# OpenPPL/ppq

Measured on AMD Instinct MI355X. Metric: calibration samples/sec (RuntimeCalibrationPass, KL 2048-bin, ResNet-50 INT8), higher is better.
Workload: dtype f32; 1 GPU; ResNet-50 topology (53 Conv + 1 Gemm, BN folded, seeded He init), RuntimeCalibrationPass kl 2048 bins, per-tensor INT8 activations, per-channel INT8 weights, 279 batches x 32 x 3x224x224 per GPU; samples=8928, batch=32, observed_tensors=72, rccl_ranks=1, async_observe=False, cache_params=False, channels_last=False, fuse_params=True, batch_observations=True, reuse_activations=False, replayed_batches=0, hip_graph=auto, graph_replays=0, miopen_find=False

## Files before the change

### include/ppq_hip.h

```cpp
#ifndef PPQ_HIP_H_
#define PPQ_HIP_H_

#include <stdint.h>

#ifdef __cplusplus
extern "C" {
#endif

typedef enum {
    PPQHIP_OK = 0,
    PPQHIP_ERR_INVALID_VALUE = -1,
    PPQHIP_ERR_UNSUPPORTED = -2,
    PPQHIP_ERR_HIP = -3
} ppqhip_status;

#define PPQHIP_ABI_VERSION 4

const char* ppqhip_last_error(void);
int ppqhip_version(void);
int ppqhip_device_arch(char* buf, int n);

int ppqhip_fq_linear_t(const float* x, const float* scale, const float* offset, float* out,
                       int64_t n, int clip_min, int clip_max, int rounding, void* stream);

// ... 49 lines not shown
    int64_t n, num_channel, elem_per_channel;
    int32_t clip_min, clip_max;
} ppqhip_lsq_job;
int ppqhip_fq_linear_c_bwd_multi(const ppqhip_lsq_job* jobs, int num_jobs, int rounding, void* stream);

int ppqhip_fq_float_t(const float* x, const float* scale, const float* offset, float* out,
                      int64_t n, int exponent, int mantissa, float clip_min, float clip_max,
                      int rounding, void* stream);

int ppqhip_fq_float_c(const float* x, const float* scale, const float* offset, float* out,
                      int64_t n, int64_t num_channel, int64_t elem_per_channel,
                      int exponent, int mantissa, float clip_min, float clip_max,
                      int rounding, void* stream);

typedef struct ppqhip_float_search_job {
    const float* x;
    int64_t rows, row_len;
    int32_t exponent, mantissa;
    float clip_min, clip_max;
} ppqhip_float_search_job;
int64_t ppqhip_float_scale_search_table_bytes(int num_jobs);
int ppqhip_float_scale_search(const ppqhip_float_search_job* jobs, int num_jobs, const float* candidates,
                              int num_candidates, int rounding, void* device_table, double* out, void* stream);

typedef struct ppqhip_fq_float_job {
    const float* x;
    const float* scale;
    const float* offset;
    float* out;
    int64_t n, num_channel, elem_per_channel;
    int32_t exponent, mantissa;
    float clip_min, clip_max;
} ppqhip_fq_float_job;
int64_t ppqhip_fq_float_multi_table_bytes(int num_jobs);
int ppqhip_fq_float_multi(const ppqhip_fq_float_job* jobs, int num_jobs, int rounding, void* device_table,
                          int upload, void* stream);

int ppqhip_fq_float_c_bwd(const float* x, const float* scale, const float* offset,
                          const float* grad_y, float* grad_x, float* grad_s, int64_t n,
                          int64_t num_channel, int64_t elem_per_channel,
                          int exponent, int mantissa, float clip_min, float clip_max,
                          int rounding, void* stream);

int64_t ppqhip_hist_workspace_bytes(int64_t n, int64_t num_bins);
int ppqhip_hist_sym_t(const float* x, int64_t n, float hist_scale, int clip_outliers,
                      int32_t* hist, int64_t num_bins, void* workspace, void* stream);

int ppqhip_hist_asym_t(const float* x, int64_t n, float min_value, float max_value,
                       int clip_outliers, int32_t* hist, int64_t num_bins, void* workspace,
                       void* stream);

int ppqhip_hist_sym_c(const float* x, int64_t n, int64_t num_channel, int64_t elem_per_channel,
                      float hist_scale, int clip_outliers, int32_t* hist, int64_t num_bins,
                      void* stream);

int ppqhip_hist_sym_c_scales(const float* x, int64_t n, int64_t num_channel, int64_t elem_per_channel,
                             const float* hist_scales, int clip_outliers, int32_t* hist,
                             int64_t num_bins, void* stream);
int ppqhip_hist_asym_c_ranges(const float* x, int64_t n, int64_t num_channel, int64_t elem_per_channel,
                              const float* mins, const float* maxs, int clip_outliers, int32_t* hist,
                              int64_t num_bins, void* stream);

int64_t ppqhip_quantile_workspace_bytes(int64_t n);
int ppqhip_quantile_t(const float* x, int64_t n, float q, float* dest, uint32_t* hint, void* workspace,
                      void* stream);

typedef struct ppqhip_quantile_job {
    const float* x;
    float* dest;
    uint32_t* hint;
    int64_t n;
} ppqhip_quantile_job;
int64_t ppqhip_quantile_multi_workspace_bytes(int num_jobs, int64_t total_elems);
int ppqhip_quantile_t_multi(const ppqhip_quantile_job* jobs, int num_jobs, float q, void* workspace,
                            void* stream);
void ppqhip_quantile_debug_layout(int64_t* out);
void ppqhip_quantile_hot_layout(int64_t* out);

int ppqhip_isotone_t(const float* x, int64_t n, float* dest, void* workspace, void* stream);

int64_t ppqhip_minmax_workspace_bytes(int64_t n);
int ppqhip_minmax_t(const float* x, int64_t n, float* minmax, void* workspace, void* stream);

int ppqhip_minmax_c(const float* x, int64_t n, int64_t num_channel, int64_t elem_per_channel,
                    float* mins, float* maxs, void* stream);

typedef struct ppqhip_minmax_c_job {
    const float* x;
    float* mins;
    float* maxs;
    int64_t n, num_channel, elem_per_channel;
    int32_t fresh, reserved;
} ppqhip_minmax_c_job;
int ppqhip_minmax_c_multi(const ppqhip_minmax_c_job* jobs, int num_jobs, void* stream);

int ppqhip_channel_sum(const float* x, int64_t n, int64_t num_channel, int64_t elem_per_channel,
                       double* sums, void* stream);

int64_t ppqhip_hist_rows(void);
int ppqhip_hist_sym_t_rows(const float* x, int64_t n, float hist_scale, int clip_outliers,
                           int32_t* rows, int64_t num_bins, void* stream);
int ppqhip_hist_asym_t_rows(const float* x, int64_t n, float min_value, float max_value,
                            int clip_outliers, int32_t* rows, int64_t num_bins, void* stream);
typedef struct ppqhip_minmax_job {
    const float* x;
    float* slots;
    int64_t n;
} ppqhip_minmax_job;
int ppqhip_minmax_t_slots_multi(const ppqhip_minmax_job* jobs, int num_jobs, void* stream);

typedef struct ppqhip_hist_job {
    const float* x;
    int32_t* rows;
    int64_t n;
    float p0, p1;
} ppqhip_hist_job;
int ppqhip_hist_t_rows_multi(const ppqhip_hist_job* jobs, int num_jobs, int asymmetric,
                             int clip_outliers, int64_t num_bins, void* stream);
int ppqhip_hist_rows_finish(const int32_t* rows, int64_t num_bins, int32_t* hist, void* stream);
int ppqhip_check_bin_rule(const float* x, int64_t n, float min_value, float hist_scale, int asymmetric, uint64_t* out, void* stream);
int64_t ppqhip_minmax_slots(void);
int ppqhip_minmax_t_slots(const float* x, int64_t n, float* slots, void* stream);
int ppqhip_minmax_slots_finish(const float* slots, float* minmax, void* stream);

float ppqhip_mse_loss_host(const int64_t* hist, int64_t num_bins, int start, int step, int end);

int64_t ppqhip_mse_search_workspace_bytes(int64_t num_hist);
int ppqhip_mse_search(const int32_t* hist, int64_t num_hist, int64_t num_bins,
                      const double* hist_scale, const double* min_value,
                      int quant_min, int quant_max, int symmetrical, int32_t* best,
                      void* workspace, void* stream);

int64_t ppqhip_kl_num_candidates(int64_t num_bins, int num_of_bits);
int ppqhip_kl_losses(const int32_t* hist, int64_t num_hist, int64_t num_bins, int num_of_bits,
                     double* losses, void* stream);

int ppqhip_tensor_clip_t(const float* value, const float* reference, const float* limit,
                         float* out, int64_t n, void* stream);
int ppqhip_tensor_clip_c(const float* value, const float* reference, const float* limit,
                         float* out, int64_t n, int64_t num_channel, int64_t elem_per_channel,
                         void* stream);
int ppqhip_rounding_loss(const float* x, const float* scale, const float* offset, float* out,
                         int64_t n, int64_t num_channel, int64_t elem_per_channel,
                         int clip_min, int clip_max, int rounding, void* stream);
int ppqhip_rounding_loss_bwd(const float* x, const float* dy, const float* scale,
                             const float* offset, float* dx, int64_t n, int64_t num_channel,
                             int64_t elem_per_channel, int clip_min, int clip_max, int rounding,
                             void* stream);

int ppqhip_bias_act(float* y, const float* bias, int64_t n, int64_t num_channel, int64_t elem_per_channel,
                    int relu, void* stream);
int ppqhip_bias_add_act(float* a, const float* bias_a, float* b, const float* bias_b, float* out,
                        int64_t n, int64_t num_channel, int64_t elem_per_channel, int relu, void* stream);

typedef struct ppqhip_adaround_job {
    const float* w;
    const float* v;
    const float* scale;
    const float* offset;
    float* out;
    const float* dy;
    int64_t n, num_channel, elem_per_channel;
    int32_t qmin, qmax;
} ppqhip_adaround_job;
int ppqhip_adaround_fwd_multi(const ppqhip_adaround_job* jobs, int num_jobs, void* stream);
int ppqhip_adaround_bwd_multi(const ppqhip_adaround_job* jobs, int num_jobs, const float* reg, void* stream);

typedef struct ppqhip_roundtune_job {
    const float* w;
    const float* r;
    const float* scale;
    const float* offset;
    float* out;
    int64_t n, num_channel, elem_per_channel;
    int32_t qmin, qmax;
} ppqhip_roundtune_job;
int ppqhip_roundtune_fwd_multi(const ppqhip_roundtune_job* jobs, int num_jobs, void* stream);

typedef struct ppqhip_fetch_rows_job {
    const float* x;
    const int32_t* index;
    float* out;
    int64_t rows, row_len, count;
} ppqhip_fetch_rows_job;
int ppqhip_fetch_rows_multi(const ppqhip_fetch_rows_job* jobs, int num_jobs, void* stream);
typedef struct ppqhip_measure_rows_job {
    const float* p;
    const float* r;
    const int32_t* index;
    double* sums;
    int64_t rows, row_len, count;
} ppqhip_measure_rows_job;
int ppqhip_measure_rows_multi(const ppqhip_measure_rows_job* jobs, int num_jobs, void* stream);
enum { PPQHIP_MEASURE_SNR = 0, PPQHIP_MEASURE_MSE = 1, PPQHIP_MEASURE_COSINE = 2 };
enum { PPQHIP_REDUCE_MEAN = 0, PPQHIP_REDUCE_MAX = 1 };
typedef struct ppqhip_measure_finish_job {
    const double* sums;
    double* acc;
    float* row_out;
    int64_t rows, count;
    int32_t method, reduce;
} ppqhip_measure_finish_job;
int ppqhip_measure_finish_multi(const ppqhip_measure_finish_job* jobs, int num_jobs, void* stream);

typedef struct ppqhip_equalize_segment {
    const float* base;
    int64_t extent;
    int64_t div, a, b;
    int64_t outer, stride, run;
    float multiplier;
    int32_t downstream;
} ppqhip_equalize_segment;
typedef struct ppqhip_equalize_scale_job {
    const ppqhip_equalize_segment* segments;
    float* scale;
    int32_t num_segments, num_channel;
    float value_threshold;
    int32_t reserved;
} ppqhip_equalize_scale_job;
int ppqhip_equalize_scale_multi(const ppqhip_equalize_scale_job* jobs, int num_jobs, void* stream);
typedef struct ppqhip_equalize_apply_job {
    float* x;
    const float* scale;
    int64_t n, run, inner, group_out;
    int64_t num_scale;
    int32_t divide, reserved;
} ppqhip_equalize_apply_job;
int ppqhip_equalize_apply_multi(const ppqhip_equalize_apply_job* jobs, int num_jobs, void* stream);

typedef struct ppqhip_split_plan_job {
    const ppqhip_equalize_segment* segments;
    int32_t* src_of;
    int32_t* count;
    int32_t num_segments, num_channel;
    float value_threshold;
    int32_t reserved;
} ppqhip_split_plan_job;
int ppqhip_split_plan_multi(const ppqhip_split_plan_job* jobs, int num_jobs, void* stream);
typedef struct ppqhip_split_apply_job {
    const float* x;
    float* out;
    const int32_t* src_of;
    int64_t n, run;
    int32_t num_channel, count;
} ppqhip_split_apply_job;
int ppqhip_split_apply_multi(const ppqhip_split_apply_job* jobs, int num_jobs, void* stream);

typedef struct ppqhip_ssd_scales_job {
    ppqhip_equalize_segment first, last;
    const float* act_range;
    float* scales;
    float* ranges;
    int32_t num_channel;
    float channel_ratio;
} ppqhip_ssd_scales_job;
int ppqhip_ssd_scales_multi(const ppqhip_ssd_scales_job* jobs, int num_jobs, void* stream);
typedef struct ppqhip_ssd_apply_job {
    const float* x;
    float* out;
    const float* scales;
    int64_t n, run, inner, group_out;
    int64_t num_channel;
    int32_t divide, reserved;
} ppqhip_ssd_apply_job;
int ppqhip_ssd_apply_multi(const ppqhip_ssd_apply_job* jobs, int num_jobs, void* stream);
typedef struct ppqhip_fq_measure_rows_job {
    const float* y;
    const float* r;
    const float* scale;
    const float* offset;
    double* sums;
    int64_t rows, count;
    int64_t num_channel, elem_per_channel;
    int32_t clip_min, clip_max, rounding, reserved;
} ppqhip_fq_measure_rows_job;
int ppqhip_fq_measure_rows_multi(const ppqhip_fq_measure_rows_job* jobs, int num_jobs, void* stream);

typedef struct ppqhip_stat_job {
    const float* p;
    const float* r;
    float* rec;
    int64_t n;
    int32_t bins, reserved;
} ppqhip_stat_job;
int ppqhip_stat_moments_multi(const ppqhip_stat_job* jobs, int num_jobs, void* stream);
int ppqhip_stat_shape_multi(const ppqhip_stat_job* jobs, int num_jobs, void* stream);

#define PPQHIP_PROF_MAX_KERNELS 40
typedef struct {
    char name[48];
    int64_t launches;
    double total_ms;
    double total_bytes;
} ppqhip_prof_entry;
int ppqhip_prof_enable(int on);
int ppqhip_prof_collect(ppqhip_prof_entry* entries, int max_entries);
double ppqhip_prof_event_overhead_us(void* stream, int pairs);

#ifdef __cplusplus
}
#endif
#endif
```

### ppq_amd/_lib.py

```python
import ctypes
import os

_HERE = os.path.dirname(os.path.abspath(__file__))
LIB_PATH = os.path.join(_HERE, 'libppq_hip.so')

c_f32p = ctypes.c_void_p
c_i32p = ctypes.c_void_p
c_f64p = ctypes.c_void_p
c_i64 = ctypes.c_int64
c_int = ctypes.c_int
c_flt = ctypes.c_float
c_vp = ctypes.c_void_p

ABI_VERSION = 4


class ProfEntry(ctypes.Structure):
    _fields_ = [('name', ctypes.c_char * 48), ('launches', ctypes.c_int64),
                ('total_ms', ctypes.c_double), ('total_bytes', ctypes.c_double)]


PROTOTYPES = {
    'ppqhip_last_error': (ctypes.c_char_p, []),
    'ppqhip_version': (c_int, []),
    'ppqhip_device_arch': (c_int, [ctypes.c_char_p, c_int]),
    'ppqhip_fq_linear_t': (c_int, [c_f32p, c_f32p, c_f32p, c_f32p, c_i64, c_int, c_int, c_int, c_vp]),
    'ppqhip_fq_linear_c': (c_int, [c_f32p, c_f32p, c_f32p, c_f32p, c_i64, c_i64, c_i64, c_int, c_int, c_int, c_vp]),
    'ppqhip_to_int_t': (c_int, [c_f32p, c_f32p, c_f32p, c_vp, c_i64, c_int, c_int, c_int, c_int, c_vp]),
    'ppqhip_to_int_c': (c_int, [c_f32p, c_f32p, c_f32p, c_vp, c_i64, c_i64, c_i64, c_int, c_int, c_int, c_int, c_vp]),
    'ppqhip_fq_linear_t_bwd': (c_int, [c_f32p, c_f32p, c_f32p, c_f32p, c_f32p, c_f32p, c_i64, c_int, c_int, c_int,
                                       c_vp]),
    'ppqhip_fq_linear_c_bwd': (c_int, [c_f32p, c_f32p, c_f32p, c_f32p, c_f32p, c_f32p, c_i64, c_i64, c_i64, c_int,
                                       c_int, c_int, c_vp]),
    'ppqhip_fq_linear_c_bwd_multi': (c_int, [c_vp, c_int, c_int, c_vp]),
    'ppqhip_fq_linear_t_bwd_partials': (c_i64, [c_i64]),
    'ppqhip_fq_linear_t_bwd_main': (c_int, [c_f32p, c_f32p, c_f32p, c_f32p, c_f32p, c_f32p, c_i64, c_int, c_int, c_int, c_vp]),
    'ppqhip_lsq_finish_multi': (c_int, [c_vp, c_int, c_vp]),
    'ppqhip_bias_act': (c_int, [c_f32p, c_f32p, c_i64, c_i64, c_i64, c_int, c_vp]),
    'ppqhip_bias_add_act': (c_int, [c_f32p, c_f32p, c_f32p, c_f32p, c_f32p, c_i64, c_i64, c_i64, c_int, c_vp]),
    'ppqhip_fq_float_t': (c_int, [c_f32p, c_f32p, c_f32p, c_f32p, c_i64, c_int, c_int, c_flt, c_flt, c_int, c_vp]),
    'ppqhip_fq_float_c': (c_int, [c_f32p, c_f32p, c_f32p, c_f32p, c_i64, c_i64, c_i64, c_int, c_int, c_flt, c_flt,
                                  c_int, c_vp]),
    'ppqhip_fq_float_c_bwd': (c_int, [c_f32p, c_f32p, c_f32p, c_f32p, c_f32p, c_f32p, c_i64, c_i64, c_i64, c_int,
                                      c_int, c_flt, c_flt, c_int, c_vp]),
    'ppqhip_hist_workspace_bytes': (c_i64, [c_i64, c_i64]),
    'ppqhip_hist_sym_t': (c_int, [c_f32p, c_i64, c_flt, c_int, c_i32p, c_i64, c_vp, c_vp]),
    'ppqhip_hist_asym_t': (c_int, [c_f32p, c_i64, c_flt, c_flt, c_int, c_i32p, c_i64, c_vp, c_vp]),
    'ppqhip_hist_sym_c': (c_int, [c_f32p, c_i64, c_i64, c_i64, c_flt, c_int, c_i32p, c_i64, c_vp]),
    'ppqhip_hist_sym_c_scales': (c_int, [c_f32p, c_i64, c_i64, c_i64, c_f32p, c_int, c_i32p, c_i64, c_vp]),
    'ppqhip_hist_asym_c_ranges': (c_int, [c_f32p, c_i64, c_i64, c_i64, c_f32p, c_f32p, c_int, c_i32p, c_i64, c_vp]),
    'ppqhip_quantile_workspace_bytes': (c_i64, [c_i64]),
    'ppqhip_quantile_t': (c_int, [c_f32p, c_i64, c_flt, c_f32p, c_vp, c_vp, c_vp]),
    'ppqhip_isotone_t': (c_int, [c_f32p, c_i64, c_f32p, c_vp, c_vp]),
    'ppqhip_minmax_workspace_bytes': (c_i64, [c_i64]),
    'ppqhip_minmax_t': (c_int, [c_f32p, c_i64, c_f32p, c_vp, c_vp]),
    'ppqhip_minmax_c': (c_int, [c_f32p, c_i64, c_i64, c_i64, c_f32p, c_f32p, c_vp]),
    'ppqhip_minmax_c_multi': (c_int, [c_vp, c_int, c_vp]),
    'ppqhip_fq_linear_multi_table_bytes': (c_i64, [c_int]),
    'ppqhip_fq_linear_multi': (c_int, [c_vp, c_int, c_int, c_vp, c_int, c_vp]),
    'ppqhip_float_scale_search_table_bytes': (c_i64, [c_int]),
    'ppqhip_float_scale_search': (c_int, [c_vp, c_int, c_vp, c_int, c_int, c_vp, c_vp, c_vp]),
    'ppqhip_fq_float_multi_table_bytes': (c_i64, [c_int]),
    'ppqhip_fq_float_multi': (c_int, [c_vp, c_int, c_int, c_vp, c_int, c_vp]),
    'ppqhip_quantile_multi_workspace_bytes': (c_i64, [c_int, c_i64]),
    'ppqhip_quantile_t_multi': (c_int, [c_vp, c_int, c_flt, c_vp, c_vp]),
    'ppqhip_quantile_debug_layout': (None, [c_vp]),
    'ppqhip_quantile_hot_layout': (None, [c_vp]),
    'ppqhip_minmax_t_slots_multi': (c_int, [c_vp, c_int, c_vp]),
    'ppqhip_hist_t_rows_multi': (c_int, [c_vp, c_int, c_int, c_int, c_i64, c_vp]),
    'ppqhip_channel_sum': (c_int, [c_f32p, c_i64, c_i64, c_i64, c_f64p, c_vp]),
    'ppqhip_hist_rows': (c_i64, []),
    'ppqhip_hist_sym_t_rows': (c_int, [c_f32p, c_i64, c_flt, c_int, c_i32p, c_i64, c_vp]),
    'ppqhip_hist_asym_t_rows': (c_int, [c_f32p, c_i64, c_flt, c_flt, c_int, c_i32p, c_i64, c_vp]),
    'ppqhip_hist_rows_finish': (c_int, [c_i32p, c_i64, c_i32p, c_vp]),
    'ppqhip_check_bin_rule': (c_int, [c_f32p, c_i64, c_flt, c_flt, c_int, c_vp, c_vp]),
    'ppqhip_minmax_slots': (c_i64, []),
    'ppqhip_minmax_t_slots': (c_int, [c_f32p, c_i64, c_f32p, c_vp]),
    'ppqhip_minmax_slots_finish': (c_int, [c_f32p, c_f32p, c_vp]),
    'ppqhip_mse_loss_host': (c_flt, [ctypes.POINTER(ctypes.c_int64), c_i64, c_int, c_int, c_int]),
    'ppqhip_mse_search_workspace_bytes': (c_i64, [c_i64]),
    'ppqhip_mse_search': (c_int, [c_i32p, c_i64, c_i64, c_f64p, c_f64p, c_int, c_int, c_int, c_i32p, c_vp, c_vp]),
    'ppqhip_kl_num_candidates': (c_i64, [c_i64, c_int]),
    'ppqhip_kl_losses': (c_int, [c_i32p, c_i64, c_i64, c_int, c_f64p, c_vp]),
    'ppqhip_tensor_clip_t': (c_int, [c_f32p, c_f32p, c_f32p, c_f32p, c_i64, c_vp]),
    'ppqhip_tensor_clip_c': (c_int, [c_f32p, c_f32p, c_f32p, c_f32p, c_i64, c_i64, c_i64, c_vp]),
    'ppqhip_rounding_loss': (c_int, [c_f32p, c_f32p, c_f32p, c_f32p, c_i64, c_i64, c_i64, c_int, c_int, c_int, c_vp]),
    'ppqhip_rounding_loss_bwd': (c_int, [c_f32p, c_f32p, c_f32p, c_f32p, c_f32p, c_i64, c_i64, c_i64, c_int, c_int,
                                         c_int, c_vp]),
    'ppqhip_adaround_fwd_multi': (c_int, [c_vp, c_int, c_vp]),
    'ppqhip_adaround_bwd_multi': (c_int, [c_vp, c_int, c_f32p, c_vp]),
    'ppqhip_roundtune_fwd_multi': (c_int, [c_vp, c_int, c_vp]),
    'ppqhip_equalize_scale_multi': (c_int, [c_vp, c_int, c_vp]),
    'ppqhip_equalize_apply_multi': (c_int, [c_vp, c_int, c_vp]),
    'ppqhip_split_plan_multi': (c_int, [c_vp, c_int, c_vp]),
    'ppqhip_split_apply_multi': (c_int, [c_vp, c_int, c_vp]),
    'ppqhip_ssd_scales_multi': (c_int, [c_vp, c_int, c_vp]),
    'ppqhip_ssd_apply_multi': (c_int, [c_vp, c_int, c_vp]),
    'ppqhip_fq_measure_rows_multi': (c_int, [c_vp, c_int, c_vp]),
    'ppqhip_fetch_rows_multi': (c_int, [c_vp, c_int, c_vp]),
    'ppqhip_measure_rows_multi': (c_int, [c_vp, c_int, c_vp]),
    'ppqhip_measure_finish_multi': (c_int, [c_vp, c_int, c_vp]),
    'ppqhip_stat_moments_multi': (c_int, [c_vp, c_int, c_vp]),
    'ppqhip_stat_shape_multi': (c_int, [c_vp, c_int, c_vp]),
    'ppqhip_prof_enable': (c_int, [c_int]),
    'ppqhip_prof_collect': (c_int, [ctypes.POINTER(ProfEntry), c_int]),
    'ppqhip_prof_event_overhead_us': (ctypes.c_double, [c_vp, c_int]),
}

if not os.path.exists(LIB_PATH):
    raise ImportError(
        f'{LIB_PATH} is missing: the HIP kernel library has not been built.  Run '
        '`python -c "import __graft_entry__ as g; g.build()"` or `make -C ppq_amd/csrc` (needs hipcc, '
        'targets gfx950).  ppq_amd has no CPU / PyTorch fallback by design.')

import torch

_torch_hip = os.path.join(os.path.dirname(torch.__file__), 'lib', 'libamdhip64.so')
if os.path.exists(_torch_hip):
    ctypes.CDLL(_torch_hip, mode=ctypes.RTLD_GLOBAL)

try:
    lib = ctypes.CDLL(LIB_PATH)
except OSError as e:
    raise ImportError(f'cannot load {LIB_PATH}: {e}') from e

for _name, (_res, _args) in PROTOTYPES.items():
    _fn = getattr(lib, _name)
    _fn.restype = _res
    _fn.argtypes = _args


if lib.ppqhip_version() != ABI_VERSION:
    raise ImportError(f'{LIB_PATH} has ABI version {lib.ppqhip_version()}, this package needs {ABI_VERSION}: rebuild it '
                      '(`make -C ppq_amd/csrc` or `python -c "import __graft_entry__ as g; g.build()"`)')


def last_error() -> str:
    msg = lib.ppqhip_last_error()
    return msg.decode('utf-8', 'replace') if msg else ''
```

### ppq_amd/calibration.py

```python
import time
from math import ceil
from typing import Callable, Dict, Iterable, List

from .core import QuantizationStates, state_value
from .distributed import merge_observers
from .observer import OperationObserver, TorchHistObserver, render_observers


class QuantizationOptimizationPass:
    def __init__(self, name: str = 'Default Quanzation Optim') -> None:
        self.name = name

    def apply(self, graph, **kwargs) -> None:
        self.optimize(graph, **kwargs)

    def optimize(self, graph, **kwargs) -> None:
        raise NotImplementedError('Implement this function first.')

    def __str__(self) -> str:
        return 'QuantizationOptimizationPass[' + self.name + ']'


class RuntimeCalibrationPass(QuantizationOptimizationPass):
    AUTO_GRAPH_ISSUE_FRACTION = 0.7
    AUTO_GRAPH_MIN_STEPS = 12

    def __init__(self, method: str = None, override: bool = False, calib_steps: int = 32,
                 process_group=None, check_steps: bool = True, async_observe: bool = False,
                 use_hip_graph: bool = False, batch_observations: bool = True,
                 reuse_activations: bool = False, reuse_budget_bytes: int = 64 << 30,
                 queue_bytes: int = None) -> None:
        super().__init__(name='PPQ Runtime Calibration Pass')
        self._method = method
        self._observers: Dict[str, OperationObserver] = {}
        self._collate_fn = None
        self._calib_steps = calib_steps
        self._override = override
        self._process_group = process_group
        self._check_steps = check_steps
        self._async_observe = async_observe
        self._use_hip_graph = use_hip_graph
        self._batch_observations = batch_observations
        self._queue = None
        self._reuse_activations = reuse_activations
        self._queue_bytes = queue_bytes
        self._reuse_budget = reuse_budget_bytes
        self._replay: list = []
        self._replay_bytes = 0
        self.replay_peak_bytes = 0
        self.replayed_batches = 0
        self._recording = False
        self.graph_replays = 0
        self.graph_decisions = []
        self.merge_stats = []
        self._side_stream = None

    def _batches(self, dataloader: Iterable) -> list:
        out = []
        for calib_epoch in range(ceil(self._calib_steps / len(dataloader))):
            for data in dataloader:
                if self._collate_fn is not None:
                    data = self._collate_fn(data)
                out.append(data)
                if len(out) >= self._calib_steps: return out
        return out

    def _graph_replayable(self, batches: list, hooks: Dict[str, object]) -> bool:
        import torch
        from .observer import ConstantObserver, TorchHistObserver, TorchMinMaxObserver, TorchMSEObserver
        if not self._use_hip_graph or len(batches) < 4: return False
        if not all(isinstance(b, torch.Tensor) and b.is_cuda and b.shape == batches[0].shape
                   and b.dtype == batches[0].dtype for b in batches): return False
        safe = (TorchMinMaxObserver, TorchHistObserver, TorchMSEObserver, ConstantObserver)
        return all(type(ob) in safe for hook in hooks.values() for ob in hook._observer_table.values())

    @ staticmethod
    def _forward_fn(executor):
        return executor.forward

    def _forward(self, executor, data, hooks, output_names):
        import torch
        recording = self._queue is not None and self._recording
        if recording: self._queue.recorder = []
        with torch.no_grad():
            self._forward_fn(executor)(inputs=data, hooks=hooks, output_names=output_names)
        if self._queue is not None: self._queue.flush()
        if recording:
            rec, self._queue.recorder = self._queue.recorder, None
            size = sum(v.numel() * 4 for _, v in rec)
            if self._replay_bytes + size <= self._reuse_budget:
                self._replay.append(rec); self._replay_bytes += size
                self.replay_peak_bytes = max(self.replay_peak_bytes, self._replay_bytes)
            else: self._recording = False

    def _replay_phase2(self, batches: list) -> int:
        n = min(len(self._replay), len(batches))
        for i in range(n):
            for ob, value in self._replay[i]: ob.observe(value)
            self._queue.flush()
            self._replay[i] = None
        self._replay, self._replay_bytes = [], 0
        self.replayed_batches += n
        return n

    def calibrate(self, desc: str, dataloader: Iterable, executor, hooks: Dict[str, object],
                  output_names: List[str] = None):
        import torch
        batches = self._batches(dataloader)
        if self._replay and not self._recording:
            batches = batches[self._replay_phase2(batches):]
            if not batches: return
        if not self._graph_replayable(batches, hooks):
            for data in batches:
                self._forward(executor, data, hooks, output_names)
            return
        self._forward(executor, batches[0], hooks, output_names)
        first = 1
        if self._use_hip_graph == 'auto':
            torch.cuda.synchronize()
            t0 = time.perf_counter()
            self._forward(executor, batches[1], hooks, output_names)
            t1 = time.perf_counter()
            torch.cuda.synchronize()
            t2 = time.perf_counter()
            first = 2
            launch_bound = (t1 - t0) > self.AUTO_GRAPH_ISSUE_FRACTION * (t2 - t0)
            self.graph_decisions.append({'phase': desc, 'issue_ms': (t1 - t0) * 1e3, 'total_ms': (t2 - t0) * 1e3,
                                         'graph': bool(launch_bound and len(batches) - first >= self.AUTO_GRAPH_MIN_STEPS)})
            if not self.graph_decisions[-1]['graph']:
                for data in batches[first:]:
                    self._forward(executor, data, hooks, output_names)
                return
        self._recording = False
        static_in = torch.empty_like(batches[0])
        torch.cuda.synchronize()
        graph = torch.cuda.CUDAGraph()
        with torch.cuda.graph(graph):
            self._forward(executor, static_in, hooks, output_names)
            if self._side_stream is not None:
                torch.cuda.current_stream().wait_stream(self._side_stream)
        for data in batches[first:]:
            static_in.copy_(data, non_blocking=True)
            graph.replay()
            self.graph_replays += 1

    def _all_tensor_observers(self):
        return [ob for op_ob in self._observers.values() for ob in op_ob.observers()]

    def _render(self):
        observers = self._all_tensor_observers()
        if self._queue is not None: self._queue.flush()
        if self._side_stream is not None:
            import torch
            torch.cuda.current_stream().wait_stream(self._side_stream)
        if merge_observers(observers, group=self._process_group):
            from . import distributed
            self.merge_stats.append(dict(distributed.last_merge_stats))
        render_observers(observers)

    def optimize(self, graph, dataloader: Iterable, executor, calib_steps: int = 32,
                 collate_fn: Callable = None, **kwargs) -> None:
        if collate_fn is not None: self._collate_fn = collate_fn
        if calib_steps is not None: self._calib_steps = calib_steps
        if self._check_steps:
            assert self._calib_steps >= 8, (
                'Insufficient Calibration Detected, to get a better quantization performance, '
                'more calibration steps is required, we strongly recommend you to prepare more calibration data '
                'and more calibration steps is preferred here. (at least 8)')
            assert self._calib_steps <= 512, (
                'Calibration steps is too large, ppq can quantize your network within 8-512 '
                'calibration steps. More calibration steps will greatly delay ppq\'s calibration procedure. '
                'Reset your calib_steps parameter please.')

        if self._override:
            for operation in graph.operations.values():
                if not hasattr(operation, 'config'): continue
                for config, var in operation.config_with_variable:
                    if (not var.is_parameter and state_value(config.state) == QuantizationStates.ACTIVATED.value
                            and config.dominated_by == config):
                        config.state = type(config.state).INITIAL

        self._observers = {}
        hooks = {}
        import torch
        if self._async_observe and torch.cuda.is_available():
            self._side_stream = torch.cuda.Stream()
        for op_name, operation in graph.operations.items():
            if not hasattr(operation, 'config'): continue
            for config, var in operation.config_with_variable:
                if not var.is_parameter and self._method is not None:
                    config.observer_algorithm = self._method
            observer = OperationObserver(operation=executor._graph.operations[op_name], monitor_parameter=False)
            observer.hook.stream = self._side_stream
            self._observers[op_name] = observer
            hooks[op_name] = observer.hook

        self._queue = None
        if self._batch_observations and self._side_stream is None:
            from .observer import ObservationQueue
            self._queue = ObservationQueue() if self._queue_bytes is None else ObservationQueue(self._queue_bytes)
        for ob in self._all_tensor_observers(): ob.queue = self._queue

        self._replay, self._replay_bytes = [], 0
        self._recording = bool(self._reuse_activations and self._queue is not None)
        self.calibrate(desc='Calibration Progress(Phase 1)', dataloader=dataloader, executor=executor,
                       hooks=hooks, output_names=None)
        self._recording = False
        self._render()
        if self._replay:
            for observer in self._observers.values():
                for cfg, ob in observer.hook._observer_table.items():
                    if (not getattr(ob._watch_on, 'is_parameter', False)
                            and QuantizationStates.is_activated(cfg.state)):
                        self._replay, self._replay_bytes = [], 0
                        break
                if not self._replay: break

        pop_list = []
        for op_name, observer in self._observers.items():
            if all([not isinstance(var_observer, TorchHistObserver)
                    for var_observer in observer.observers()]):
                pop_list.append(op_name)
        for op_name in pop_list:
            self._observers.pop(op_name)
            hooks.pop(op_name)

        if len(hooks) > 0:
            self.calibrate(desc='Calibration Progress(Phase 2)', dataloader=dataloader, executor=executor,
                           hooks=hooks, output_names=None)
            self._render()


class PPLDSPTIReCalibrationPass(RuntimeCalibrationPass):
    def __init__(self, method: str = None, override: bool = False) -> None:
        super().__init__(method, override)
        self.name = 'PPQ ReCalibration For Computing Op Pass'

    def optimize(self, graph, dataloader: Iterable, executor, calib_steps: int, collate_fn: Callable = None, **kwargs) -> None:
        from .blocks import COMPUTING_OP, downstream_operations
        from .core import QuantizationPolicy, QuantizationProperty as P, TensorQuantizationConfig
        from .observer import CalibrationHook, TensorObserverFactroy, TorchMinMaxObserver
        self._collate_fn, self._calib_steps = collate_fn, calib_steps
        assert calib_steps >= 8, ('Insufficient Calibration Detected, to better quantize your network, more calibration steps is '
                                  'demonded, we strongly recommend you to prepare more calibration data and more calibration '
                                  'steps is preferred here. (at least 8)')
        assert calib_steps <= 512, ('Calibration steps is too large, ppq is capable for quantizing your network within 32-128 '
                                    'calibration steps. More calibraiton steps will greatly delay ppq\'s calibration procedure. '
                                    'Reset your calib_steps parameter please.')

        def probe(like, per_channel: bool, consumer):
            bits = P.SYMMETRICAL.value + P.LINEAR.value + (P.PER_CHANNEL.value if per_channel else P.PER_TENSOR.value)
            return TensorQuantizationConfig(policy=QuantizationPolicy(bits), rounding=like.rounding, num_of_bits=like.num_of_bits,
                                            quant_min=like.quant_min, quant_max=like.quant_max, scale=None, offset=None,
                                            observer_algorithm='Minmax', state=QuantizationStates.INITIAL,
                                            channel_axis=1 if per_channel else None, detail={'consumer': consumer})
        hooks = {}
        for operation in graph.topological_sort():
            if not hasattr(operation, 'config') or operation.type not in COMPUTING_OP: continue
            output_cfg = operation.config.output_quantization_config[0]
            master_cfg, master_operation, master_var = output_cfg, operation, operation.outputs[0]
            table = {}
            if operation.inputs[0].name in graph.inputs:
                input_cfg = operation.config.input_quantization_config[0]
                table[input_cfg] = TensorObserverFactroy.build_observer(operation.inputs[0], probe(input_cfg, False, input_cfg))
            followers = downstream_operations(operation)
            if len(followers) == 1 and followers[0].type in {'Relu', 'Clip'} and hasattr(followers[0], 'config'):
                if table:
                    hooks[operation.name] = CalibrationHook(operation, table)
                    table = {}
                master_operation = followers[0]
                master_cfg = master_operation.config.output_quantization_config[0]
                master_var = master_operation.outputs[0]
            table[master_cfg] = TensorObserverFactroy.build_observer(master_var, probe(master_cfg, True, output_cfg))
            assert master_operation.name not in hooks, 'register an operation in calibration hooks twice'
            hooks[master_operation.name] = CalibrationHook(master_operation, table)

        self._queue = None
        self.calibrate(desc='ReCalibration For Computing Ops', dataloader=dataloader, executor=executor, hooks=hooks)

        for hook in hooks.values():
            for observer in hook._observer_table.values():
                cfg = observer._quant_cfg.detail['consumer']
                assert isinstance(observer, TorchMinMaxObserver)
                r = observer._range_on_host()
                if observer._quant_cfg.policy.has_property(P.PER_CHANNEL):
                    cfg.detail.update({'range_min': r[0].copy(), 'range_max': r[1].copy()})
                else:
                    cfg.detail.update({'range_min': (float(r[0]),), 'range_max': (float(r[1]),)})


class IsotoneCalibrationPass(RuntimeCalibrationPass):
    def __init__(self, variables: List[str] = None, axis: int = -1, verbose: bool = True, calib_steps: int = 32) -> None:
        super().__init__(calib_steps=calib_steps)
        self.name = 'Isotone Calibration Pass'
        self.variables = variables
        self.axis = axis
        self.verbose = verbose

    @ staticmethod
    def _mark(cfg, axis: int) -> None:
        from .core import OBSERVER_ISOTONE_OBSERVER_AXIS
        cfg.state = type(cfg.state).INITIAL
        cfg.observer_algorithm = 'Isotone'
        cfg.detail[OBSERVER_ISOTONE_OBSERVER_AXIS] = axis

    def optimize(self, graph, **kwargs) -> None:
        if self.variables is None:
            for op in graph.operations.values():
                if op.type != 'Softmax' or not hasattr(op, 'config'): continue
                cfg = op.config.output_quantization_config[0]
                if cfg.dominated_by != cfg: continue
                axis = op.attributes.get('axis', -1)
                self._mark(cfg, axis)
                if self.verbose: print(f'Calibration Method of Op {op.name} has been changed to Isotone[axis={axis}].')
# ... 15 lines not shown
```

### ppq_amd/csrc/common.hpp

```cpp
#pragma once

#include <hip/hip_runtime.h>
#include <stdint.h>

#include "../../include/ppq_hip.h"

namespace ppqhip {

constexpr int kWave = 64;
constexpr int kNumCU = 256;
int num_cu();
constexpr int kBlock = 256;

enum Rounding : int {
    ROUND_HALF_EVEN = 0, ROUND_HALF_UP = 1, ROUND_HALF_DOWN = 2, ROUND_HALF_TOWARDS_ZERO = 3,
    ROUND_HALF_FAR_FORM_ZERO = 4, ROUND_TO_NEAR_INT = 5, ROUND_UP = 6, ROUND_DOWN = 7
};

void set_error(const char* fmt, ...);
int check_hip(hipError_t e, const char* what);

enum KernelId : int {
    K_FQ_LINEAR_T = 0, K_FQ_LINEAR_C, K_FQ_LINEAR_T_BWD, K_FQ_LINEAR_C_BWD, K_FQ_FLOAT_T, K_FQ_FLOAT_C,
    K_FQ_FLOAT_BWD, K_HIST_SYM_T, K_HIST_ASYM_T, K_HIST_SYM_C, K_QUANTILE, K_ISOTONE, K_MINMAX_T,
    K_MINMAX_C, K_MSE_SEARCH, K_KL_LOSSES, K_TENSOR_CLIP, K_ROUNDING_LOSS, K_CHANNEL_SUM, K_FLOAT_SCALE_SEARCH, K_LSQ_FINISH,
    K_ADAROUND_FWD, K_ADAROUND_BWD, K_FETCH_ROWS, K_MEASURE_ROWS, K_MEASURE_FINISH, K_ROUNDTUNE_FWD, K_EQUALIZE_SCALE,
    K_EQUALIZE_APPLY, K_SSD_SCALES, K_SSD_APPLY, K_FQ_MEASURE_ROWS, K_STAT_MOMENTS, K_STAT_SHAPE,
    K_SPLIT_PLAN, K_SPLIT_APPLY, K_NUM
};
extern const char* const kKernelNames[K_NUM];

struct LaunchScope {
    LaunchScope(KernelId id, double bytes, hipStream_t stream);
    ~LaunchScope();
    int slot;
    hipStream_t stream;
};

int finish_launch(const char* what);
void* scratch(hipStream_t stream, size_t bytes);
constexpr size_t kZeroedArenaBytes = 32 * 16384 * sizeof(int);
void* zeroed_arena(hipStream_t stream, size_t bytes);

inline bool aligned16(const void* p) { return (reinterpret_cast<uintptr_t>(p) & 15u) == 0; }

struct FastDiv {
    uint32_t d, m, l;
};
inline FastDiv make_fastdiv(uint32_t d) {
    FastDiv f; f.d = d; f.l = 0;
    while ((1ull << f.l) < d) f.l++;
    f.m = (uint32_t)(((1ull << 32) * ((1ull << f.l) - d)) / d + 1);
    return f;
}

#if defined(__HIPCC__)

__device__ __forceinline__ uint32_t fdiv(uint32_t n, FastDiv f) {
    return (__umulhi(n, f.m) + n) >> f.l;
}

__device__ __forceinline__ void even_split(uint32_t T, uint32_t G, uint32_t g, uint32_t& begin, uint32_t& end) {
    const uint32_t q = T / G, rem = T - q * G;
    begin = g * q + min(g, rem);
    end = begin + q + (g < rem ? 1u : 0u);
}

__device__ __forceinline__ int f2i_sat(float v) {
    int r;
    asm("v_cvt_i32_f32 %0, %1" : "=v"(r) : "v"(v));
    return r;
}
__device__ __forceinline__ int d2i_sat(double v) {
    int r;
    asm("v_cvt_i32_f64 %0, %1" : "=v"(r) : "v"(v));
    return r;
}

__device__ __forceinline__ int add_sat(int a, int b) { return __builtin_elementwise_add_sat(a, b); }

__device__ __forceinline__ int clampi(int v, int lo, int hi) { return v > hi ? hi : (v < lo ? lo : v); }

template <int R>
__device__ __forceinline__ int round2int_t(float value) {
    if constexpr (R == ROUND_HALF_EVEN) return f2i_sat(__builtin_rintf(value));
    else if constexpr (R == ROUND_HALF_UP) return d2i_sat(__builtin_floor((double)value + .5));
    else if constexpr (R == ROUND_HALF_DOWN) return d2i_sat(__builtin_ceil((double)value - .5));
    else if constexpr (R == ROUND_HALF_TOWARDS_ZERO)
        return value > 0 ? round2int_t<ROUND_HALF_DOWN>(value) : round2int_t<ROUND_HALF_UP>(value);
    else if constexpr (R == ROUND_HALF_FAR_FORM_ZERO)
        return value > 0 ? round2int_t<ROUND_HALF_UP>(value) : round2int_t<ROUND_HALF_DOWN>(value);
    else if constexpr (R == ROUND_UP) return f2i_sat(__builtin_ceilf(value));
    else if constexpr (R == ROUND_DOWN) return f2i_sat(__builtin_floorf(value));
    else return f2i_sat(__builtin_roundf(value));
}

__device__ __forceinline__ int round2int(float value, int rounding) {
    switch (rounding) {
        case ROUND_HALF_EVEN: return round2int_t<ROUND_HALF_EVEN>(value);
        case ROUND_HALF_UP: return round2int_t<ROUND_HALF_UP>(value);
        case ROUND_HALF_DOWN: return round2int_t<ROUND_HALF_DOWN>(value);
        case ROUND_HALF_TOWARDS_ZERO: return round2int_t<ROUND_HALF_TOWARDS_ZERO>(value);
        case ROUND_HALF_FAR_FORM_ZERO: return round2int_t<ROUND_HALF_FAR_FORM_ZERO>(value);
        case ROUND_UP: return round2int_t<ROUND_UP>(value);
        case ROUND_DOWN: return round2int_t<ROUND_DOWN>(value);
        default: return round2int_t<ROUND_TO_NEAR_INT>(value);
    }
}

__device__ __forceinline__ int round_offset(float o) { return f2i_sat(__builtin_roundf(o)); }

template <int R>
__device__ __forceinline__ float fq_linear_scalar(float x, float s, int o, int qmin, int qmax, int rounding) {
    const float qt = x / s;
    const int r = (R >= 0) ? round2int_t<(R >= 0 ? R : 0)>(qt) : round2int(qt, rounding);
    const int q = clampi(add_sat(r, o), qmin, qmax);
    return (float)(q - o) * s;
}

__device__ __forceinline__ float fq_safe_rcp(float s) {
    const float a = __builtin_fabsf(s);
    return (a >= 0x1p-100f && a <= 0x1p100f) ? __builtin_amdgcn_rcpf(s) : __builtin_nanf("");
}
__device__ __forceinline__ float rne_tie_margin(float t, float d) {
    return __builtin_fmaf(__builtin_fabsf(t), 0x1p-20f, __builtin_fabsf(d));
}

template <int R>
__device__ __forceinline__ void round_quotient4(const float4& a, float s, float rc, int rounding, int (&r)[4]) {
    if constexpr (R == ROUND_HALF_EVEN) {
        typedef float pk2 __attribute__((ext_vector_type(2)));
        const pk2 t01 = pk2{a.x, a.y} * rc, t23 = pk2{a.z, a.w} * rc;
        float r0 = __builtin_rintf(t01.x), r1 = __builtin_rintf(t01.y), r2 = __builtin_rintf(t23.x), r3 = __builtin_rintf(t23.y);
        const pk2 d01 = t01 - pk2{r0, r1}, d23 = t23 - pk2{r2, r3};
        const float m0 = rne_tie_margin(t01.x, d01.x), m1 = rne_tie_margin(t01.y, d01.y);
        const float m2 = rne_tie_margin(t23.x, d23.x), m3 = rne_tie_margin(t23.y, d23.y);
        if (!(__builtin_fmaxf(__builtin_fmaxf(m0, m1), __builtin_fmaxf(m2, m3)) <= 0.5f)) {
            if (!(m0 <= 0.5f)) r0 = __builtin_rintf(a.x / s);
            if (!(m1 <= 0.5f)) r1 = __builtin_rintf(a.y / s);
            if (!(m2 <= 0.5f)) r2 = __builtin_rintf(a.z / s);
            if (!(m3 <= 0.5f)) r3 = __builtin_rintf(a.w / s);
        }
        r[0] = f2i_sat(r0); r[1] = f2i_sat(r1); r[2] = f2i_sat(r2); r[3] = f2i_sat(r3);
    } else {
        r[0] = (R >= 0) ? round2int_t<(R >= 0 ? R : 0)>(a.x / s) : round2int(a.x / s, rounding);
        r[1] = (R >= 0) ? round2int_t<(R >= 0 ? R : 0)>(a.y / s) : round2int(a.y / s, rounding);
        r[2] = (R >= 0) ? round2int_t<(R >= 0 ? R : 0)>(a.z / s) : round2int(a.z / s, rounding);
        r[3] = (R >= 0) ? round2int_t<(R >= 0 ? R : 0)>(a.w / s) : round2int(a.w / s, rounding);
    }
}

template <int R>
__device__ __forceinline__ float4 fq_linear4(const float4& a, float s, float rc, int o, int qmin, int qmax, int rounding) {
    int r[4];
    round_quotient4<R>(a, s, rc, rounding, r);
    float4 out;
    out.x = (float)(clampi(add_sat(r[0], o), qmin, qmax) - o) * s;
    out.y = (float)(clampi(add_sat(r[1], o), qmin, qmax) - o) * s;
    out.z = (float)(clampi(add_sat(r[2], o), qmin, qmax) - o) * s;
    out.w = (float)(clampi(add_sat(r[3], o), qmin, qmax) - o) * s;
    return out;
}

__device__ __forceinline__ float wave_min(float v) {
#pragma unroll
    for (int m = 32; m > 0; m >>= 1) v = fminf(v, __shfl_xor(v, m, 64));
    return v;
}
__device__ __forceinline__ float wave_max(float v) {
#pragma unroll
    for (int m = 32; m > 0; m >>= 1) v = fmaxf(v, __shfl_xor(v, m, 64));
    return v;
}
__device__ __forceinline__ float wave_sum(float v) {
#pragma unroll
    for (int m = 32; m > 0; m >>= 1) v += __shfl_xor(v, m, 64);
    return v;
}

__device__ __forceinline__ void atomic_min_f32(float* addr, float v) {
    if (__float_as_int(v) >= 0) atomicMin(reinterpret_cast<int*>(addr), __float_as_int(v));
// ... 216 lines not shown
```

### ppq_amd/csrc/epilogue.hip

```cpp
#include "common.hpp"

namespace ppqhip {
namespace {

constexpr int kEpTileU = 2;
constexpr int kEpSmallU = 1;
constexpr long long kEpSmallElems = 1ll << 20;

struct EpArgs {
    float* a;
    const float* bias_a;
    float* b;
    const float* bias_b;
    float* out;
    uint32_t nvec;
    uint32_t tail;
    int ntail;
    FastDiv epc;
    FastDiv nc;
};

__device__ __forceinline__ uint32_t channel_of(uint32_t i, const FastDiv& epc, const FastDiv& nc) {
    const uint32_t row = fdiv(i, epc);
    return row - fdiv(row, nc) * nc.d;
}

__device__ __forceinline__ float act(float v, bool relu) {
    return (relu && !__builtin_isnan(v)) ? __builtin_fmaxf(v, 0.f) : v;
}

__device__ __forceinline__ float4 add4(const float4& x, const float4& y) {
    return make_float4(x.x + y.x, x.y + y.y, x.z + y.z, x.w + y.w);
}

template <bool RELU>
__device__ __forceinline__ float4 act4(const float4& v) {
    return make_float4(act(v.x, RELU), act(v.y, RELU), act(v.z, RELU), act(v.w, RELU));
}

template <bool PLANE>
__device__ __forceinline__ float4 bias4(const float* __restrict__ bias, uint32_t v, const FastDiv& epc, const FastDiv& nc) {
    if (PLANE) {
        const float t = bias[channel_of(v, epc, nc)];
        return make_float4(t, t, t, t);
    }
    const uint32_t i = v * 4u;
    return make_float4(bias[channel_of(i, epc, nc)], bias[channel_of(i + 1, epc, nc)], bias[channel_of(i + 2, epc, nc)],
                       bias[channel_of(i + 3, epc, nc)]);
}

template <bool RESID, bool BIAS_B, bool RELU>
__device__ __forceinline__ void epilogue_elem(const EpArgs& p, uint32_t i, const FastDiv& epc) {
    const uint32_t c = channel_of(i, epc, p.nc);
    const float x = p.a[i] + p.bias_a[c];
    if (!RESID) { p.a[i] = act(x, RELU); return; }
    p.a[i] = x;
    float y = p.b[i];
    if (BIAS_B) { y = y + p.bias_b[c]; p.b[i] = y; }
    p.out[i] = act(x + y, RELU);
}

template <int U, bool RESID, bool BIAS_B, bool RELU, bool PLANE>
__global__ __launch_bounds__(kBlock) void epilogue_kernel(EpArgs p) {
    const uint32_t base = blockIdx.x * (kBlock * U) + threadIdx.x;
    float4* a4 = reinterpret_cast<float4*>(p.a);
    float4* b4 = reinterpret_cast<float4*>(p.b);
    float4* o4 = reinterpret_cast<float4*>(p.out);
    float4 a[U], ba[U], b[U], bb[U];
#pragma unroll
    for (int k = 0; k < U; k++) {
        const uint32_t vv = min(base + k * kBlock, p.nvec - 1);
        a[k] = a4[vv];
        ba[k] = bias4<PLANE>(p.bias_a, vv, p.epc, p.nc);
        if (RESID) b[k] = b4[vv];
        if (BIAS_B) bb[k] = bias4<PLANE>(p.bias_b, vv, p.epc, p.nc);
    }
#pragma unroll
    for (int k = 0; k < U; k++) {
        const uint32_t vv = base + k * kBlock;
        if (vv >= p.nvec) continue;
        const float4 x = add4(a[k], ba[k]);
        if (!RESID) { a4[vv] = act4<RELU>(x); continue; }
        a4[vv] = x;
        float4 y = b[k];
        if (BIAS_B) { y = add4(y, bb[k]); b4[vv] = y; }
        o4[vv] = act4<RELU>(add4(x, y));
    }
    if (!PLANE && blockIdx.x == 0 && (int)threadIdx.x < p.ntail)
        epilogue_elem<RESID, BIAS_B, RELU>(p, p.tail + threadIdx.x, p.epc);
}

template <bool RESID, bool BIAS_B, bool RELU>
__global__ __launch_bounds__(kBlock) void epilogue_scalar_kernel(EpArgs p) {
    const uint32_t stride = gridDim.x * kBlock;
    for (uint32_t i = blockIdx.x * kBlock + threadIdx.x; i < (uint32_t)p.ntail; i += stride)
        epilogue_elem<RESID, BIAS_B, RELU>(p, i, p.epc);
}

template <bool RESID, bool BIAS_B, bool RELU>
void launch_epilogue(EpArgs p, int64_t n, int64_t C, int64_t epc, bool aligned, hipStream_t st) {
    p.nc = make_fastdiv((uint32_t)C);
    if (!aligned || n < 4) {
        p.nvec = 0; p.tail = 0; p.ntail = (int)n;
        p.epc = make_fastdiv((uint32_t)epc);
        hipLaunchKernelGGL((epilogue_scalar_kernel<RESID, BIAS_B, RELU>), dim3(stream_grid(n, kBlock)), dim3(kBlock), 0, st, p);
        return;
    }
    p.nvec = (uint32_t)(n >> 2);
    p.tail = p.nvec * 4u;
    p.ntail = (int)(n & 3);
    const bool plane = (epc % 4 == 0);
    p.epc = make_fastdiv((uint32_t)(plane ? epc / 4 : epc));
#define PPQ_LAUNCH_EP(U, PLANE)                                                                                          \
    hipLaunchKernelGGL((epilogue_kernel<U, RESID, BIAS_B, RELU, PLANE>), dim3((p.nvec + kBlock * U - 1) / (kBlock * U)),   \
                       dim3(kBlock), 0, st, p)
    if (n <= kEpSmallElems) {
        if (plane) PPQ_LAUNCH_EP(kEpSmallU, true); else PPQ_LAUNCH_EP(kEpSmallU, false);
    } else {
        if (plane) PPQ_LAUNCH_EP(kEpTileU, true); else PPQ_LAUNCH_EP(kEpTileU, false);
    }
#undef PPQ_LAUNCH_EP
}

int validate(int64_t n, int64_t C, int64_t epc, const char* what) {
    if (n <= 0 || n > 0x7fffffffLL) {
        set_error("%s: n=%lld is empty or has more than 2^31 - 1 elements", what, (long long)n);
        return PPQHIP_ERR_INVALID_VALUE;
    }
    if (C <= 0 || epc <= 0 || C > 0x7fffffffLL || epc > 0x7fffffffLL || n % (C * epc) != 0) {
        set_error("%s: n=%lld is not [outer, %lld channels, %lld elem/channel]", what, (long long)n, (long long)C,
                  (long long)epc);
        return PPQHIP_ERR_INVALID_VALUE;
    }
    return PPQHIP_OK;
}

}
}

using namespace ppqhip;

extern "C" {

int ppqhip_bias_act(float* y, const float* bias, int64_t n, int64_t num_channel, int64_t elem_per_channel, int relu,
                    void* stream) {
    if (int st = validate(n, num_channel, elem_per_channel, "bias_act")) return st;
    if (!y || !bias) { set_error("bias_act: null pointer"); return PPQHIP_ERR_INVALID_VALUE; }
    hipStream_t s = (hipStream_t)stream;
    EpArgs p{};
    p.a = y; p.bias_a = bias;
    const bool aligned = aligned16(y);
    if (relu) launch_epilogue<false, false, true>(p, n, num_channel, elem_per_channel, aligned, s);
    else launch_epilogue<false, false, false>(p, n, num_channel, elem_per_channel, aligned, s);
    return finish_launch("bias_act");
}

int ppqhip_bias_add_act(float* a, const float* bias_a, float* b, const float* bias_b, float* out, int64_t n,
                        int64_t num_channel, int64_t elem_per_channel, int relu, void* stream) {
    if (int st = validate(n, num_channel, elem_per_channel, "bias_add_act")) return st;
    if (!a || !bias_a || !b || !out) { set_error("bias_add_act: null pointer"); return PPQHIP_ERR_INVALID_VALUE; }
    hipStream_t s = (hipStream_t)stream;
    EpArgs p{};
    p.a = a; p.bias_a = bias_a; p.b = b; p.bias_b = bias_b; p.out = out;
    const bool aligned = aligned16(a) && aligned16(b) && aligned16(out);
    if (bias_b) {
        if (relu) launch_epilogue<true, true, true>(p, n, num_channel, elem_per_channel, aligned, s);
        else launch_epilogue<true, true, false>(p, n, num_channel, elem_per_channel, aligned, s);
    } else {
        if (relu) launch_epilogue<true, false, true>(p, n, num_channel, elem_per_channel, aligned, s);
        else launch_epilogue<true, false, false>(p, n, num_channel, elem_per_channel, aligned, s);
    }
    return finish_launch("bias_add_act");
}

}
```

### ppq_amd/csrc/hist.hip

```cpp
#include "common.hpp"

namespace ppqhip {

constexpr int kMaxLdsBins = 16384;
constexpr int kLdsBudgetInts = 2048;
constexpr int kHistBlock = 512;
constexpr int kHistWgPerCu = 2;
constexpr int kHistU = 2;
constexpr int kHistMinTiles = 2;
constexpr int kHistAtomicMaxWg = 128;
constexpr long long kHistNtElems = 48ll << 20;
constexpr int kHistRows = kNumCU * kHistWgPerCu;
constexpr uint32_t kTileVec = (uint32_t)kHistBlock * kHistU;
constexpr uint32_t kTileElems = kTileVec * 4;
static_assert(kHistBlock % 64 == 0 && kHistBlock >= 64 && kHistBlock <= 1024, "histogram workgroup: whole waves");

typedef float v2f __attribute__((ext_vector_type(2)));

struct BinRule {
    float a;
    float hs;
    float rcp;
    int bins;
    int clip;
    int asym;
};
static BinRule make_rule(float a, float hs, int bins, int clip, int asym) {
    BinRule r; r.a = a; r.hs = hs; r.rcp = 1.0f / hs; r.bins = bins; r.clip = clip; r.asym = asym;
    return r;
}

__device__ __forceinline__ bool quotient_is_safe(float t) {
    return __builtin_fabsf(t - __builtin_rintf(t)) >= __builtin_fabsf(t) * 0x1p-22f;
}

__device__ __forceinline__ int f2i_abs(float t) {
    int r;
    asm("v_cvt_i32_f32_e64 %0, |%1|" : "=v"(r) : "v"(t));
    return r;
}
__device__ __forceinline__ int f2i_floor(float t) {
    int r;
    asm("v_cvt_flr_i32_f32 %0, %1" : "=v"(r) : "v"(t));
    return r;
}

template <bool ASYM, bool CLIP, bool HOT>
struct Binner : WaveBinCounter<ASYM, CLIP, HOT> {
    using Base = WaveBinCounter<ASYM, CLIP, HOT>;
    using Base::h; using Base::last; using Base::hot_bin; using Base::hot_cnt;
    float a0, hs, rcp;

    __device__ __forceinline__ void set_rule(float a, float scale) { a0 = a; hs = scale; rcp = 1.0f / scale; }

    __device__ __forceinline__ void bins4(const float4& v, int (&b)[4]) const {
        v2f x01 = {v.x, v.y}, x23 = {v.z, v.w};
        if (ASYM) { x01 = x01 - a0; x23 = x23 - a0; }
        const v2f t01 = x01 * rcp, t23 = x23 * rcp;
        const v2f r01 = {__builtin_rintf(t01.x), __builtin_rintf(t01.y)};
        const v2f r23 = {__builtin_rintf(t23.x), __builtin_rintf(t23.y)};
        const v2f d01 = t01 - r01, d23 = t23 - r23;
        const v2f e01 = t01 * 0x1p-22f, e23 = t23 * 0x1p-22f;
        const bool u0 = !(__builtin_fabsf(d01.x) >= __builtin_fabsf(e01.x));
        const bool u1 = !(__builtin_fabsf(d01.y) >= __builtin_fabsf(e01.y));
        const bool u2 = !(__builtin_fabsf(d23.x) >= __builtin_fabsf(e23.x));
        const bool u3 = !(__builtin_fabsf(d23.y) >= __builtin_fabsf(e23.y));
        b[0] = ASYM ? f2i_floor(t01.x) : f2i_abs(t01.x);
        b[1] = ASYM ? f2i_floor(t01.y) : f2i_abs(t01.y);
        b[2] = ASYM ? f2i_floor(t23.x) : f2i_abs(t23.x);
        b[3] = ASYM ? f2i_floor(t23.y) : f2i_abs(t23.y);
        if (u0 | u1 | u2 | u3) {
            if (u0) b[0] = exact_bin(ASYM ? x01.x : __builtin_fabsf(v.x));
            if (u1) b[1] = exact_bin(ASYM ? x01.y : __builtin_fabsf(v.y));
            if (u2) b[2] = exact_bin(ASYM ? x23.x : __builtin_fabsf(v.z));
            if (u3) b[3] = exact_bin(ASYM ? x23.y : __builtin_fabsf(v.w));
        }
    }
    __device__ __forceinline__ int exact_bin(float a) const { return f2i_sat(__builtin_floorf(a / hs)); }

    __device__ __forceinline__ int bin1(float v) const {
        const float a = ASYM ? (v - a0) : __builtin_fabsf(v);
        const float t = a * rcp;
        if (quotient_is_safe(t)) return ASYM ? f2i_floor(t) : f2i_abs(t);
        return exact_bin(a);
    }

};

constexpr int kReduceBins = 32, kReduceSlices = 32, kReduceBlock = kReduceBins * kReduceSlices;
__global__ __launch_bounds__(kReduceBlock) void hist_reduce_kernel(const int* __restrict__ partial, int count, int bins,
                                                                   int* __restrict__ hist) {
    __shared__ int lds[kReduceSlices][kReduceBins];
    const int lane_bin = threadIdx.x % kReduceBins, slice = threadIdx.x / kReduceBins;
    const int b = blockIdx.x * kReduceBins + lane_bin;
    int total = 0;
    if (b < bins) {
        int i = slice;
        for (; i + 15 * kReduceSlices < count; i += 16 * kReduceSlices) {
            int v[16];
#pragma unroll
            for (int k = 0; k < 16; k++) v[k] = partial[(size_t)(i + k * kReduceSlices) * bins + b];
#pragma unroll
            for (int k = 0; k < 16; k++) total += v[k];
        }
        for (; i < count; i += kReduceSlices) total += partial[(size_t)i * bins + b];
    }
    lds[slice][lane_bin] = total;
    __syncthreads();
    if (slice == 0 && b < bins) {
        int t = 0;
#pragma unroll
        for (int k = 0; k < kReduceSlices; k++) t += lds[k][lane_bin];
        if (t) hist[b] += t;
    }
}

constexpr int kMultiMax = 96;
enum FlushMode : int {
    FLUSH_ROWS_ADD = 0,
    FLUSH_ROWS_STORE = 1,
    FLUSH_ATOMIC = 2
};
struct HistJob {
    const float* x;
    int* rows;
    uint32_t n;
    float a, hs;
    uint32_t first_tile;
};
struct HistJobs {
    HistJob job[kMultiMax];
    uint32_t count;
    uint32_t total_tiles;
    int bins, copies, mode;
};
__host__ __device__ inline uint32_t job_tiles(uint32_t n, bool vec_ok) {
    if (!vec_ok) return (n + kTileElems - 1) / kTileElems;
    const uint32_t full = (n >> 2) / kTileVec;
    return full + (n > full * kTileElems ? 1u : 0u);
}

__device__ __forceinline__ void lds_hist_flush(int* lds, int bins, int copies, int* __restrict__ dst, int mode) {
    asm volatile("s_waitcnt lgkmcnt(0)" ::: "memory");
    __syncthreads();
    for (int b = threadIdx.x; b < bins; b += kHistBlock) {
        int s = 0;
        for (int c = 0; c < copies; c++) { s += lds[c * bins + b]; lds[c * bins + b] = 0; }
        if (mode == FLUSH_ROWS_STORE) dst[b] = s;
        else if (s) {
            if (mode == FLUSH_ROWS_ADD) dst[b] += s;
            else atomicAdd(&dst[b], s);
        }
    }
    __syncthreads();
}

template <bool ASYM, bool CLIP, bool HOT, bool NT>
__global__ __launch_bounds__(kHistBlock, (kHistBlock * kHistWgPerCu + 255) / 256)
void hist_persistent_kernel(const HistJobs jobs) {
    extern __shared__ int lds[];
    const uint32_t G = gridDim.x, g = blockIdx.x;
    uint32_t t, t_end;
    even_split(jobs.total_tiles, G, g, t, t_end);
    const int bins = jobs.bins, copies = jobs.copies;
    bool zeroed = false;
    auto zero_lds = [&]() {
        if (zeroed) return;
        for (int i = threadIdx.x; i < copies * bins; i += kHistBlock) lds[i] = 0;
        asm volatile("s_waitcnt lgkmcnt(0)\n\ts_barrier" ::: "memory");
        zeroed = true;
    };
    if (t >= t_end) {
        if (jobs.mode == FLUSH_ROWS_STORE) for (int b = threadIdx.x; b < bins; b += kHistBlock) jobs.job[0].rows[(size_t)g * bins + b] = 0;
        return;
    }
    uint32_t lo = 0, hi = jobs.count;
    while (hi - lo > 1) {
        const uint32_t mid = (lo + hi) >> 1;
        if (jobs.job[mid].first_tile <= t) lo = mid; else hi = mid;
    }
    Binner<ASYM, CLIP, HOT> acc;
    acc.init(lds + ((threadIdx.x >> 6) % copies) * bins, bins);

    for (uint32_t j = lo; t < t_end; j++) {
        const HistJob& job = jobs.job[j];
        const uint32_t j_end = (j + 1 < jobs.count) ? jobs.job[j + 1].first_tile : jobs.total_tiles;
        uint32_t k = t - job.first_tile;
        const uint32_t k1 = min(t_end, j_end) - job.first_tile;
        t = min(t_end, j_end);
        acc.set_rule(job.a, job.hs);
        const float* __restrict__ x = job.x;
        const uint32_t n = job.n;
        const bool vec_ok = (reinterpret_cast<uintptr_t>(x) & 15u) == 0;
        const uint32_t full = vec_ok ? (n >> 2) / kTileVec : 0u;
        const uint32_t kf = min(k1, full);
        if (k < kf) {
            const float4* xv = reinterpret_cast<const float4*>(x) + threadIdx.x;
            float4 bufa[kHistU], bufb[kHistU];
            auto fetch = [&](float4 (&buf)[kHistU], uint32_t tile) {
                const float4* p = xv + (size_t)tile * kTileVec;
#pragma unroll
                for (int u = 0; u < kHistU; u++) buf[u] = load4<NT>(p + u * kHistBlock);
            };
            auto consume = [&](const float4 (&buf)[kHistU], uint32_t tile) {
#pragma unroll
                for (int u = 0; u < kHistU; u++) {
                    int b[4];
                    acc.bins4(buf[u], b);
                    if (u == 0) acc.elect(b[0], true);
                    if (CLIP && HOT) acc.commit4_exec(b);
                    else {
                        acc.template commit<true>(b[0], true); acc.template commit<true>(b[1], true);
                        acc.template commit<true>(b[2], true); acc.template commit<true>(b[3], true);
                    }
                }
            };
            fetch(bufa, k);
            zero_lds();
            for (;;) {
                fetch(bufb, min(k + 1, kf - 1));
                consume(bufa, k);
                if (++k >= kf) break;
                fetch(bufa, min(k + 1, kf - 1));
                consume(bufb, k);
                if (++k >= kf) break;
            }
        }
        zero_lds();
        for (; k < k1; k++) {
            const uint32_t e0 = k * kTileElems + threadIdx.x;
#pragma unroll 4
            for (int r = 0; r < 4 * kHistU; r++) {
                const uint32_t i = e0 + r * kHistBlock;
                const bool in = i < n;
                const float a = in ? x[i] : 0.f;
                const int b = acc.bin1(a);
                if ((r & 3) == 0) acc.elect(b, in);
                acc.template commit<false>(b, in);
            }
        }
// ... 659 lines not shown
```

### ppq_amd/csrc/runtime.hip

```cpp
#include <cstdarg>
#include <cstdio>
#include <cstring>
#include <map>
#include <mutex>
#include <vector>

#include "common.hpp"

namespace ppqhip {

static thread_local char g_err[512] = "";

void set_error(const char* fmt, ...) {
    va_list ap;
    va_start(ap, fmt);
    vsnprintf(g_err, sizeof(g_err), fmt, ap);
    va_end(ap);
}

int check_hip(hipError_t e, const char* what) {
    if (e == hipSuccess) return PPQHIP_OK;
    set_error("HIP failure in %s: %s", what, hipGetErrorString(e));
    return PPQHIP_ERR_HIP;
}

int finish_launch(const char* what) { return check_hip(hipGetLastError(), what); }

const char* const kKernelNames[K_NUM] = {
    "fq_linear_t", "fq_linear_c", "fq_linear_t_bwd", "fq_linear_c_bwd", "fq_float_t", "fq_float_c",
    "fq_float_bwd", "hist_sym_t", "hist_asym_t", "hist_sym_c", "quantile_t", "isotone_t", "minmax_t",
    "minmax_c", "mse_search", "kl_losses", "tensor_clip", "rounding_loss", "channel_sum", "float_scale_search", "lsq_finish",
    "adaround_fwd", "adaround_bwd", "fetch_rows", "measure_rows", "measure_finish", "roundtune_fwd", "equalize_scale",
    "equalize_apply", "ssd_scales", "ssd_apply", "fq_measure_rows", "stat_moments", "stat_shape",
    "split_plan", "split_apply"};

int num_cu() {
    static std::mutex mu;
    static std::map<int, int> per_device;
    int dev = 0;
    if (hipGetDevice(&dev) != hipSuccess) return kNumCU;
    std::lock_guard<std::mutex> lk(mu);
    auto it = per_device.find(dev);
    if (it != per_device.end()) return it->second;
    int n = 0;
    if (hipDeviceGetAttribute(&n, hipDeviceAttributeMultiprocessorCount, dev) != hipSuccess || n <= 0) n = kNumCU;
    if (n > kNumCU) n = kNumCU;
    per_device[dev] = n;
    return n;
}

static std::mutex g_scratch_mu;
static std::map<std::pair<int, hipStream_t>, std::pair<void*, size_t>> g_scratch;

void* scratch(hipStream_t stream, size_t bytes) {
    int dev = 0;
    if (hipGetDevice(&dev) != hipSuccess) return nullptr;
    std::lock_guard<std::mutex> lk(g_scratch_mu);
    auto& slot = g_scratch[{dev, stream}];
    if (slot.second < bytes) {
        hipStreamCaptureStatus cap = hipStreamCaptureStatusNone;
        if (stream != nullptr && hipStreamIsCapturing(stream, &cap) == hipSuccess && cap != hipStreamCaptureStatusNone) {
            set_error("scratch: %zu bytes needed on a stream that is being captured (run the same work once eagerly on this stream first)", bytes);
            return nullptr;
        }
        if (slot.first) {
            if (hipStreamSynchronize(stream) != hipSuccess) return nullptr;
            (void)hipFree(slot.first);
            slot = {nullptr, 0};
        }
        size_t want = bytes < (1u << 20) ? (1u << 20) : bytes;
        void* p = nullptr;
        if (hipMalloc(&p, want) != hipSuccess) { set_error("scratch: hipMalloc(%zu) failed", want); return nullptr; }
        slot = {p, want};
    }
    return slot.first;
}

static std::map<std::pair<int, hipStream_t>, void*> g_zeroed;
void* zeroed_arena(hipStream_t stream, size_t bytes) {
    if (bytes > kZeroedArenaBytes) { set_error("zeroed_arena: %zu bytes asked of a %zu-byte arena", bytes, (size_t)kZeroedArenaBytes); return nullptr; }
    int dev = 0;
    if (hipGetDevice(&dev) != hipSuccess) return nullptr;
    std::lock_guard<std::mutex> lk(g_scratch_mu);
    void*& p = g_zeroed[{dev, stream}];
    if (p == nullptr) {
        hipStreamCaptureStatus cap = hipStreamCaptureStatusNone;
        if (stream != nullptr && hipStreamIsCapturing(stream, &cap) == hipSuccess && cap != hipStreamCaptureStatusNone) return nullptr;
        void* q = nullptr;
        if (hipMalloc(&q, kZeroedArenaBytes) != hipSuccess) { set_error("zeroed_arena: hipMalloc failed"); return nullptr; }
        if (hipMemset(q, 0, kZeroedArenaBytes) != hipSuccess) { (void)hipFree(q); set_error("zeroed_arena: hipMemset failed"); return nullptr; }
        p = q;
    }
    return p;
}

struct ProfRecord {
    int id;
    double bytes;
    hipEvent_t start, stop;
};
static std::mutex g_prof_mu;
static bool g_prof_on = false;
static std::vector<ProfRecord> g_records;
static std::vector<hipEvent_t> g_pool;

static hipEvent_t get_event() {
    if (!g_pool.empty()) { hipEvent_t e = g_pool.back(); g_pool.pop_back(); return e; }
    hipEvent_t e; (void)hipEventCreate(&e); return e;
}

LaunchScope::LaunchScope(KernelId id, double bytes, hipStream_t s) : slot(-1), stream(s) {
    if (!g_prof_on) return;
    hipStreamCaptureStatus cap = hipStreamCaptureStatusNone;
    if (s != nullptr && hipStreamIsCapturing(s, &cap) == hipSuccess && cap != hipStreamCaptureStatusNone) return;
    std::lock_guard<std::mutex> lk(g_prof_mu);
    ProfRecord r; r.id = id; r.bytes = bytes; r.start = get_event(); r.stop = get_event();
    (void)hipEventRecord(r.start, stream);
    g_records.push_back(r);
    slot = (int)g_records.size() - 1;
}

LaunchScope::~LaunchScope() {
    if (slot < 0) return;
    std::lock_guard<std::mutex> lk(g_prof_mu);
    (void)hipEventRecord(g_records[slot].stop, stream);
}

}

using namespace ppqhip;

extern "C" {

const char* ppqhip_last_error(void) { return g_err; }

int ppqhip_version(void) { return PPQHIP_ABI_VERSION; }

int ppqhip_device_arch(char* buf, int n) {
    int dev = 0;
    if (int st = check_hip(hipGetDevice(&dev), "hipGetDevice")) return st;
    hipDeviceProp_t prop;
    if (int st = check_hip(hipGetDeviceProperties(&prop, dev), "hipGetDeviceProperties")) return st;
    snprintf(buf, n, "%s", prop.gcnArchName);
    return PPQHIP_OK;
}

int ppqhip_prof_enable(int on) {
    std::lock_guard<std::mutex> lk(g_prof_mu);
    g_prof_on = on != 0;
    return PPQHIP_OK;
}

double ppqhip_prof_event_overhead_us(void* stream, int pairs) {
    hipStream_t s = (hipStream_t)stream;
    if (pairs < 1) pairs = 1;
    std::vector<hipEvent_t> ev(2 * (size_t)pairs);
    for (auto& e : ev) if (hipEventCreate(&e) != hipSuccess) return -1.0;
    for (int i = 0; i < pairs; i++) {
        (void)hipEventRecord(ev[2 * i], s);
        (void)hipEventRecord(ev[2 * i + 1], s);
    }
    (void)hipStreamSynchronize(s);
    double total = 0.0;
    for (int i = 0; i < pairs; i++) {
        float ms = 0.f;
        (void)hipEventElapsedTime(&ms, ev[2 * i], ev[2 * i + 1]);
        total += ms;
    }
    for (auto& e : ev) (void)hipEventDestroy(e);
    return total * 1e3 / pairs;
}

int ppqhip_prof_collect(ppqhip_prof_entry* entries, int max_entries) {
    std::lock_guard<std::mutex> lk(g_prof_mu);
    ppqhip_prof_entry agg[K_NUM];
    memset(agg, 0, sizeof(agg));
    for (int k = 0; k < K_NUM; k++) snprintf(agg[k].name, sizeof(agg[k].name), "%s", kKernelNames[k]);
    for (auto& r : g_records) {
        float ms = 0.f;
        (void)hipEventSynchronize(r.stop);
        (void)hipEventElapsedTime(&ms, r.start, r.stop);
        agg[r.id].launches += 1; agg[r.id].total_ms += ms; agg[r.id].total_bytes += r.bytes;
        g_pool.push_back(r.start); g_pool.push_back(r.stop);
    }
    g_records.clear();
    int n = 0;
    for (int k = 0; k < K_NUM && n < max_entries; k++)
// ... 6 lines not shown
```

### ppq_amd/ffi.py

```python
import threading
import weakref
from typing import List

import numpy as np
import torch

from . import _lib
from ._lib import lib

_KERNEL_FAILURE = 'Kernel Failure, '


_raw_stream = torch._C._cuda_getCurrentRawStream
_get_device = torch._C._cuda_getDevice


def _stream() -> int:
    return _raw_stream(_get_device())


def _check(t: torch.Tensor, dtype: torch.dtype, name: str) -> None:
    if not isinstance(t, torch.Tensor):
        raise TypeError(f'{name}: expected a torch.Tensor, got {type(t)}')
    if t.dtype != dtype:
        raise RuntimeError(_KERNEL_FAILURE + 'Invalid dtype of Input tensor: ' + name)
    if t.numel() == 0:
        raise RuntimeError(_KERNEL_FAILURE + 'Tensor is empty: ' + name)
    if not t.is_cuda:
        raise RuntimeError(_KERNEL_FAILURE + f'{name} is not on the GPU (ppq_amd has no CPU path)')


_F32 = torch.float32


def _f32(t, name):
    try:
        if t.dtype is _F32 and t.is_cuda and t.numel() > 0: return
    except AttributeError:
        pass
    _check(t, torch.float32, name + '(Expect to be FP32)')


def _dense(t: torch.Tensor, channel_axis=None) -> torch.Tensor:
    if t.is_contiguous(): return t
    if channel_axis is None or channel_axis % t.dim() == 0:
        if t.dim() == 4 and t.is_contiguous(memory_format=torch.channels_last): return t
        if t.dim() == 5 and t.is_contiguous(memory_format=torch.channels_last_3d): return t
    return t.contiguous()


def _raise(status: int) -> None:
    if status != 0:
        raise RuntimeError(_KERNEL_FAILURE + _lib.last_error())


def _geometry(shape, channel_axis: int):
    ndim = len(shape)
    if channel_axis < 0: channel_axis += ndim
    if not 0 <= channel_axis < ndim:
        raise RuntimeError(_KERNEL_FAILURE + f'channel_axis {channel_axis} out of range for a {ndim}-d tensor')
    epc = 1
    for d in shape[channel_axis + 1:]:
        epc *= int(d)
    return int(shape[channel_axis]), epc


class _DeviceOf:
    __slots__ = ('idx', 'prev')

    def __init__(self, t: torch.Tensor):
        self.idx = t.device.index
        self.prev = None

    def __enter__(self):
        if self.idx is not None and self.idx != _get_device():
            self.prev = _get_device()
            torch.cuda.set_device(self.idx)

    def __exit__(self, *a):
        if self.prev is not None:
            torch.cuda.set_device(self.prev)


_workspaces = {}
_MAX_WORKSPACES = 16


def _workspace(device: torch.device, nbytes: int) -> torch.Tensor:
    key = (device.index, _stream())
    ws = _workspaces.pop(key, None)
    if ws is None or ws.numel() < nbytes:
        ws = torch.empty(max(nbytes, 1 << 16), dtype=torch.uint8, device=device)
    _workspaces[key] = ws
    while len(_workspaces) > _MAX_WORKSPACES:
        _workspaces.pop(next(iter(_workspaces)))
    return ws


_MINMAX_JOB = np.dtype([('x', '<u8'), ('slots', '<u8'), ('n', '<i8')])
_FQ_JOB = np.dtype([('x', '<u8'), ('scale', '<u8'), ('offset', '<u8'), ('out', '<u8'), ('n', '<i8'),
                    ('num_channel', '<i8'), ('elem_per_channel', '<i8'), ('clip_min', '<i4'), ('clip_max', '<i4')])
_FQ_FLOAT_JOB = np.dtype([('x', '<u8'), ('scale', '<u8'), ('offset', '<u8'), ('out', '<u8'), ('n', '<i8'),
                          ('num_channel', '<i8'), ('elem_per_channel', '<i8'), ('exponent', '<i4'), ('mantissa', '<i4'),
                          ('clip_min', '<f4'), ('clip_max', '<f4')])
_FLOAT_SEARCH_JOB = np.dtype([('x', '<u8'), ('rows', '<i8'), ('row_len', '<i8'), ('exponent', '<i4'), ('mantissa', '<i4'),
                              ('clip_min', '<f4'), ('clip_max', '<f4')])
_LSQ_JOB = np.dtype([('x', '<u8'), ('scale', '<u8'), ('offset', '<u8'), ('grad_y', '<u8'), ('grad_x', '<u8'), ('grad_s', '<u8'),
                     ('n', '<i8'), ('num_channel', '<i8'), ('elem_per_channel', '<i8'), ('clip_min', '<i4'), ('clip_max', '<i4')])
_LSQ_FINISH_JOB = np.dtype([('partial', '<u8'), ('grad_s', '<u8'), ('n', '<i8'), ('clip_min', '<i4'), ('clip_max', '<i4')])
_MINMAX_C_JOB = np.dtype([('x', '<u8'), ('mins', '<u8'), ('maxs', '<u8'), ('n', '<i8'), ('num_channel', '<i8'),
                          ('elem_per_channel', '<i8'), ('fresh', '<i4'), ('reserved', '<i4')])
_QUANTILE_JOB = np.dtype([('x', '<u8'), ('dest', '<u8'), ('hint', '<u8'), ('n', '<i8')])

_owner_hints = weakref.WeakKeyDictionary()
_hint_owner = threading.local()


def quantile_hint(device: torch.device) -> torch.Tensor:
    return torch.zeros(8, dtype=torch.int32, device=device)


class quantile_hint_owner:
    __slots__ = ('owner', 'prev')

    def __init__(self, owner):
        self.owner, self.prev = owner, None

    def __enter__(self):
        self.prev = getattr(_hint_owner, 'current', None)
        _hint_owner.current = self.owner
        return self

    def __exit__(self, *a):
        _hint_owner.current = self.prev


def _owner_quantile_hint(device: torch.device, numel: int, q: float):
    owner = getattr(_hint_owner, 'current', None)
    if owner is None: return None
    try: per = _owner_hints.setdefault(owner, {})
    except TypeError: return None
    key = (device.index, int(numel), float(q))
    h = per.get(key)
    if h is None: h = per[key] = quantile_hint(device)
    return h


_HIST_JOB = np.dtype([('x', '<u8'), ('rows', '<u8'), ('n', '<i8'), ('p0', '<f4'), ('p1', '<f4')])


def _epilogue_geometry(ts, bias_list):
    t0 = ts[0]
    if not isinstance(t0, torch.Tensor) or t0.dtype is not _F32 or not t0.is_cuda or t0.dim() != 4 or t0.numel() == 0:
        return None
    shape, strides, dev = t0.shape, t0.stride(), t0.device
    for t in ts[1:]:
        if not isinstance(t, torch.Tensor) or t.dtype is not _F32 or t.device != dev or t.shape != shape or t.stride() != strides:
            return None
    C = int(shape[1])
    for bias in bias_list:
        if (not isinstance(bias, torch.Tensor) or bias.dtype is not _F32 or bias.device != dev or bias.dim() != 1
                or bias.numel() != C or not bias.is_contiguous()):
            return None
    if t0.is_contiguous(): return C, int(shape[2]) * int(shape[3])
    if t0.is_contiguous(memory_format=torch.channels_last): return C, 1
    return None


def bias_act_(y: torch.Tensor, bias: torch.Tensor, relu: bool) -> bool:
    geo = _epilogue_geometry([y], [bias])
    if geo is None: return False
    with _DeviceOf(y):
        _raise(lib.ppqhip_bias_act(y.data_ptr(), bias.data_ptr(), y.numel(), geo[0], geo[1], 1 if relu else 0, _stream()))
    return True


def bias_add_act(a: torch.Tensor, bias_a: torch.Tensor, b: torch.Tensor, bias_b, relu: bool):
    geo = _epilogue_geometry([a, b], [bias_a] if bias_b is None else [bias_a, bias_b])
    if geo is None or a.data_ptr() == b.data_ptr(): return None
    out = torch.empty_like(a)
    with _DeviceOf(a):
        _raise(lib.ppqhip_bias_add_act(a.data_ptr(), bias_a.data_ptr(), b.data_ptr(), 0 if bias_b is None else bias_b.data_ptr(),
                                       out.data_ptr(), a.numel(), geo[0], geo[1], 1 if relu else 0, _stream()))
    return out


_ADAROUND_JOB = np.dtype([('w', '<u8'), ('v', '<u8'), ('scale', '<u8'), ('offset', '<u8'), ('out', '<u8'), ('dy', '<u8'),
                          ('n', '<i8'), ('num_channel', '<i8'), ('elem_per_channel', '<i8'), ('qmin', '<i4'), ('qmax', '<i4')])


def _adaround_table(items, outs, dys=None):
    n = len(items)
    if len(outs) != n or (dys is not None and len(dys) != n):
        raise RuntimeError(_KERNEL_FAILURE + 'AdaRound: argument lists differ in length')
    jobs = np.zeros(n, dtype=_ADAROUND_JOB)
    dev = items[0][0].device
    for k, (w, v, s, o, axis, qmin, qmax) in enumerate(items):
        ts = [('Value', w), ('Rounding', v), ('Scale', s), ('Offset', o), ('Out', outs[k])] + ([('Dy', dys[k])] if dys is not None else [])
        for name, t in ts:
            _f32(t, name)
            if t.device != dev: raise RuntimeError(_KERNEL_FAILURE + f'AdaRound: item {k}: {name} is on another device')
            if not t.is_contiguous(): raise RuntimeError(_KERNEL_FAILURE + f'AdaRound: item {k}: {name} is not contiguous')
        for name, t in ts[1:2] + ts[4:]:
            if t.shape != w.shape: raise RuntimeError(_KERNEL_FAILURE + f'AdaRound: item {k}: {name} is not shaped like the weight')
        C, epc = _geometry(w.shape, axis) if axis is not None else (1, w.numel())
        if s.numel() != C or o.numel() != C:
            raise RuntimeError(_KERNEL_FAILURE + f'AdaRound: item {k}: scale / offset need {C} elements')
        jobs[k] = (w.data_ptr(), v.data_ptr(), s.data_ptr(), o.data_ptr(), outs[k].data_ptr(),
                   dys[k].data_ptr() if dys is not None else 0, w.numel(), C, epc, int(qmin), int(qmax))
    return jobs


def adaround_forward_multi(items, outs=None) -> List[torch.Tensor]:
    if not items: return []
    if outs is None: outs = [torch.empty_like(it[0]) for it in items]
    jobs = _adaround_table(items, outs)
    with _DeviceOf(items[0][0]):
        _raise(lib.ppqhip_adaround_fwd_multi(jobs.ctypes.data, len(items), _stream()))
    return outs


def adaround_backward_multi(items, dys, reg: torch.Tensor, dvs=None) -> List[torch.Tensor]:
    if not items: return []
    _f32(reg, 'Reg')
    if reg.numel() != 3 or not reg.is_contiguous() or reg.device != items[0][0].device:
        raise RuntimeError(_KERNEL_FAILURE + 'AdaRound: reg must be a contiguous float32[3] on the weights\' device')
    if dvs is None: dvs = [torch.empty_like(it[0]) for it in items]
    jobs = _adaround_table(items, dvs, dys)
    with _DeviceOf(items[0][0]):
        _raise(lib.ppqhip_adaround_bwd_multi(jobs.ctypes.data, len(items), reg.data_ptr(), _stream()))
    return dvs


_ROUNDTUNE_JOB = np.dtype([('w', '<u8'), ('r', '<u8'), ('scale', '<u8'), ('offset', '<u8'), ('out', '<u8'),
                           ('n', '<i8'), ('num_channel', '<i8'), ('elem_per_channel', '<i8'), ('qmin', '<i4'), ('qmax', '<i4')])


def _roundtune_table(items, outs):
    n = len(items)
    if len(outs) != n: raise RuntimeError(_KERNEL_FAILURE + 'RoundTuning: argument lists differ in length')
    jobs = np.zeros(n, dtype=_ROUNDTUNE_JOB)
    dev = items[0][0].device
    for k, (w, r, s, o, axis, qmin, qmax) in enumerate(items):
        ts = [('Value', w), ('Rounding', r), ('Scale', s), ('Offset', o), ('Out', outs[k])]
        for name, t in ts:
            _f32(t, name)
            if t.device != dev: raise RuntimeError(_KERNEL_FAILURE + f'RoundTuning: item {k}: {name} is on another device')
            if not t.is_contiguous(): raise RuntimeError(_KERNEL_FAILURE + f'RoundTuning: item {k}: {name} is not contiguous')
        for name, t in ts[1:2] + ts[4:]:
            if t.shape != w.shape: raise RuntimeError(_KERNEL_FAILURE + f'RoundTuning: item {k}: {name} is not shaped like the weight')
        C, epc = _geometry(w.shape, axis) if axis is not None else (1, w.numel())
        if s.numel() != C or o.numel() != C:
            raise RuntimeError(_KERNEL_FAILURE + f'RoundTuning: item {k}: scale / offset need {C} elements')
        jobs[k] = (w.data_ptr(), r.data_ptr(), s.data_ptr(), o.data_ptr(), outs[k].data_ptr(), w.numel(), C, epc, int(qmin), int(qmax))
    return jobs


def roundtune_forward_multi(items, outs=None) -> List[torch.Tensor]:
    if not items: return []
    if outs is None: outs = [torch.empty_like(it[0]) for it in items]
    jobs = _roundtune_table(items, outs)
    with _DeviceOf(items[0][0]):
        _raise(lib.ppqhip_roundtune_fwd_multi(jobs.ctypes.data, len(items), _stream()))
    return outs


_EQ_SEGMENT = np.dtype([('base', '<u8'), ('extent', '<i8'), ('div', '<i8'), ('a', '<i8'), ('b', '<i8'), ('outer', '<i8'),
                        ('stride', '<i8'), ('run', '<i8'), ('multiplier', '<f4'), ('downstream', '<i4')])
_EQ_SCALE_JOB = np.dtype([('segments', '<u8'), ('scale', '<u8'), ('num_segments', '<i4'), ('num_channel', '<i4'),
                          ('value_threshold', '<f4'), ('reserved', '<i4')])
_EQ_APPLY_JOB = np.dtype([('x', '<u8'), ('scale', '<u8'), ('n', '<i8'), ('run', '<i8'), ('inner', '<i8'), ('group_out', '<i8'),
                          ('num_scale', '<i8'), ('divide', '<i4'), ('reserved', '<i4')])


def _eq_tensor(t, what: str, k: int, dev):
    _f32(t, what)
    if t.device != dev: raise RuntimeError(_KERNEL_FAILURE + f'Equalization: item {k}: {what} is on another device')
    if not t.is_contiguous(): raise RuntimeError(_KERNEL_FAILURE + f'Equalization: item {k}: {what} is not contiguous')


class EqualizeTable:
    __slots__ = ('jobs', 'segments', 'keep', 'entry')

    def __init__(self, jobs, segments, keep, entry):
        self.jobs, self.segments, self.keep, self.entry = jobs, segments, keep, entry

    def __len__(self) -> int: return len(self.jobs)

    def run(self) -> None:
        if len(self.jobs) == 0: return
        with _DeviceOf(self.keep[0]):
            _raise(self.entry(self.jobs.ctypes.data, len(self.jobs), _stream()))


def equalize_scale_table(items) -> EqualizeTable:
    jobs = np.zeros(len(items), dtype=_EQ_SCALE_JOB)
    segs = np.zeros(sum(len(it[2]) for it in items), dtype=_EQ_SEGMENT)
    keep, at = [], 0
    dev = items[0][0].device if items else None
    for k, (scale, threshold, segments) in enumerate(items):
        _eq_tensor(scale, 'Scale', k, dev)
        keep.append(scale)
        jobs[k] = (segs.ctypes.data + at * _EQ_SEGMENT.itemsize, scale.data_ptr(), len(segments), scale.numel(), float(threshold), 0)
        for t, div, a, b, outer, stride, run, mult, down in segments:
            _eq_tensor(t, 'Value', k, dev)
            keep.append(t)
            segs[at] = (t.data_ptr(), t.numel(), int(div), int(a), int(b), int(outer), int(stride), int(run), float(mult), 1 if down else 0)
            at += 1
    return EqualizeTable(jobs, segs, keep, lib.ppqhip_equalize_scale_multi)


def equalize_apply_table(items) -> EqualizeTable:
    jobs = np.zeros(len(items), dtype=_EQ_APPLY_JOB)
    keep = []
    dev = items[0][0].device if items else None
    for k, (x, scale, run, inner, group_out, divide) in enumerate(items):
        _eq_tensor(x, 'Value', k, dev); _eq_tensor(scale, 'Scale', k, dev)
        keep += [x, scale]
        jobs[k] = (x.data_ptr(), scale.data_ptr(), x.numel(), int(run), int(inner), int(group_out), scale.numel(), 1 if divide else 0, 0)
    return EqualizeTable(jobs, None, keep, lib.ppqhip_equalize_apply_multi)


def equalize_scale_multi(items) -> None:
    (items if isinstance(items, EqualizeTable) else equalize_scale_table(items)).run()


def equalize_apply_multi(items) -> None:
    (items if isinstance(items, EqualizeTable) else equalize_apply_table(items)).run()


_SPLIT_PLAN_JOB = np.dtype([('segments', '<u8'), ('src_of', '<u8'), ('count', '<u8'), ('num_segments', '<i4'), ('num_channel', '<i4'),
                            ('value_threshold', '<f4'), ('reserved', '<i4')])
_SPLIT_APPLY_JOB = np.dtype([('x', '<u8'), ('out', '<u8'), ('src_of', '<u8'), ('n', '<i8'), ('run', '<i8'), ('num_channel', '<i4'),
                             ('count', '<i4')])
SPLIT_MAX_JOBS, SPLIT_MAX_SEGMENTS = 32, 72
SPLIT_BIT = -0x80000000

# ... 1284 lines not shown
```

### ppq_amd/harness.py

```python
from typing import Callable, Dict, List, Optional

import torch
import torch.nn.functional as F

from .core import LinearQuantizationConfig, QuantizationStates, TensorQuantizationConfig, is_initial
from .core import QuantizationProperty as P
from .qfunction import PPQuantFunction

PASSIVE_OPERATIONS = {'MaxPool', 'GlobalMaxPool', 'Reshape', 'Flatten', 'Identity', 'Dropout', 'Slice', 'Pad', 'Resize',
                      'Split', 'Transpose', 'Interp', 'Squeeze', 'Unsqueeze'}
COMPUTING_OP = {'Conv', 'Gemm', 'ConvTranspose', 'MatMul'}


class Variable:
    def __init__(self, name: str, value: torch.Tensor = None, is_parameter: bool = False):
        self.name = name
        self.value = value
        self.stored_value = None
        self.is_parameter = is_parameter
        self.dest_ops: List['Operation'] = []
        self.source_op: Optional['Operation'] = None

    def __hash__(self): return hash(self.name)
    def __eq__(self, o): return isinstance(o, Variable) and o.name == self.name


class OperationQuantizationConfig:
    def __init__(self, input_quantization_configs, output_quantization_configs):
        self.input_quantization_config: List[TensorQuantizationConfig] = input_quantization_configs
        self.output_quantization_config: List[TensorQuantizationConfig] = output_quantization_configs


class Operation:
    def __init__(self, name: str, op_type: str, attributes: dict = None, inputs=None, outputs=None):
        self.name, self.type = name, op_type
        self.attributes = attributes or {}
        self.inputs: List[Variable] = inputs or []
        self.outputs: List[Variable] = outputs or []

    @ property
    def parameters(self) -> List[Variable]:
        return [v for v in self.inputs if v.is_parameter]

    def __str__(self): return f'{self.name}({self.type})'


class QuantableOperation(Operation):
    def __init__(self, op: Operation, config: OperationQuantizationConfig):
        super().__init__(op.name, op.type, op.attributes, op.inputs, op.outputs)
        self.config = config
        self.store_parameter_value()

    def store_parameter_value(self):
        for var in self.inputs:
            if var.is_parameter and isinstance(var.value, torch.Tensor): var.stored_value = var.value.detach().clone()
        return self

    def _swap_parameters(self) -> None:
        for var in self.inputs:
            if var.is_parameter and isinstance(var.value, torch.Tensor) and var.stored_value is not None:
                parked = var.value
                var.value = var.stored_value.to(parked.device)
                var.stored_value = parked

    @ property
    def config_with_variable(self):
        return list(zip(self.config.input_quantization_config, self.inputs)) + \
            list(zip(self.config.output_quantization_config, self.outputs))

    def dequantize(self):
        if getattr(self, '_dequantized', False): return self
        for cfg, _ in self.config_with_variable:
            cfg.detail['Stored State'] = cfg.state
            cfg.state = QuantizationStates.FP32
        self._swap_parameters()
        self._dequantized = True
        return self

    def restore_quantize_state(self):
        if not getattr(self, '_dequantized', False): return self
        for cfg, _ in self.config_with_variable:
            if 'Stored State' in cfg.detail: cfg.state = cfg.detail.pop('Stored State')
        self._swap_parameters()
        self._dequantized = False
        return self

    def baking_parameters(self, quant_func: Callable):
        for config, var in self.config_with_variable:
            if var.is_parameter and QuantizationStates.is_activated(config.state):
                var.value = quant_func(var.value, config)
                config.state = (QuantizationStates.BAKED if config.state == QuantizationStates.ACTIVATED
                                else QuantizationStates.PASSIVE_BAKED)


class BaseGraph:
    def __init__(self, name: str):
        self.name = name
        self.operations: Dict[str, Operation] = {}
        self.variables: Dict[str, Variable] = {}
        self.inputs: Dict[str, Variable] = {}
        self.outputs: Dict[str, Variable] = {}

    def create_variable(self, name: str, value=None, is_parameter=False) -> Variable:
        v = Variable(name, value, is_parameter)
        self.variables[name] = v
        return v

    def create_operation(self, op_type: str, name: str, inputs: List[Variable], attributes: dict = None) -> Variable:
        out = self.create_variable(name + '_out')
        op = Operation(name, op_type, attributes, list(inputs), [out])
        out.source_op = op
        for v in inputs: v.dest_ops.append(op)
        self.operations[name] = op
        return out

    def topological_sort(self) -> List[Operation]:
        return list(self.operations.values())


def _forward(op: Operation, x: List[torch.Tensor]):
    t, a = op.type, op.attributes
    if t == 'Conv':
        return F.conv2d(x[0], x[1], x[2] if len(x) > 2 else None, stride=a.get('strides', 1),
                        padding=a.get('pads', 0), groups=a.get('group', 1))
    if t == 'Gemm': return F.linear(x[0], x[1], x[2] if len(x) > 2 else None)
    if t == 'MatMul': return torch.matmul(x[0], x[1])
    if t == 'Relu': return F.relu(x[0])
    if t == 'Gelu': return F.gelu(x[0])
    if t == 'Add': return x[0] + x[1]
    if t == 'MaxPool': return F.max_pool2d(x[0], a['kernel_shape'], a.get('strides', 1), a.get('pads', 0))
    if t == 'GlobalAveragePool': return F.adaptive_avg_pool2d(x[0], 1)
    if t == 'Flatten': return torch.flatten(x[0], 1)
    if t == 'LayerNormalization': return F.layer_norm(x[0], x[0].shape[-1:], x[1], x[2])
    if t == 'Softmax': return F.softmax(x[0], dim=a.get('axis', -1))
    if t == 'Mul': return x[0] * (x[1] if len(x) > 1 else a['value'])
    if t == 'Reshape': return x[0].reshape(a['shape'])
    if t == 'Transpose': return x[0].permute(a['perm'])
    if t == 'Concat': return torch.cat([v.expand(x[-1].shape[0], *v.shape[1:]) if v.shape[0] == 1 else v for v in x],
                                       dim=a.get('axis', 1))
    if t == 'Slice': return x[0].narrow(a['axis'], a['start'], a['length'])
    if t == 'Resize': return F.interpolate(x[0], scale_factor=a.get('scale', 2), mode=a.get('mode', 'nearest'))
    raise NotImplementedError(f'Graph op: {op.name}({op.type}) has no backend implementation')


class EpilogueGroup:
    __slots__ = ('kind', 'ops', 'convs', 'add', 'relu')

    def __init__(self, kind, ops, convs, add, relu):
        self.kind, self.ops, self.convs, self.add, self.relu = kind, ops, convs, add, relu

    def __repr__(self): return f'{self.kind}({", ".join(op.name for op in self.ops)})'


def _in_cfg(op, i):
    return op.config.input_quantization_config[i] if isinstance(op, QuantableOperation) else None


def _out_cfg(op, i):
    return op.config.output_quantization_config[i] if isinstance(op, QuantableOperation) else None


def plan_epilogues(operations: List[Operation], hooks: Dict[str, object] = None, keep=(), passes_through: Callable = None,
                   grad_enabled: bool = False) -> List[EpilogueGroup]:
    if grad_enabled: return []
    from .observer import CalibrationHook
    hooks = hooks or {}
    keep = set(keep)
    if passes_through is None:
        def passes_through(c): return not QuantizationStates.is_activated(c.state)

    def through(*cfgs): return all(c is None or passes_through(c) for c in cfgs)

    def hooks_ok(members, unwritten):
        for op in members:
            h = hooks.get(op.name)
            if h is None: continue
            if type(h) is not CalibrationHook: return False
            if any(c is not None and c in h._observer_table for c in unwritten): return False
        return True

    def conv_ok(op):
        return (op.type == 'Conv' and len(op.inputs) == 3 and op.inputs[2].is_parameter and len(op.outputs) == 1
                and op.outputs[0].name not in keep)

    def only_feeds(v, op): return len(v.dest_ops) == 1 and v.dest_ops[0] is op

    def relu_after(op, i):
        if i >= len(operations): return None
        r = operations[i]
        out = op.outputs[0]
        if r.type != 'Relu' or len(r.inputs) != 1 or r.inputs[0] is not out or not only_feeds(out, r) or out.name in keep:
            return None
        return r

    def try_p2(i):
        for n_conv in (2, 1):
            j = i + n_conv
            if j + 1 >= len(operations): continue
            add, convs = operations[j], operations[i:j]
            if add.type != 'Add' or len(add.inputs) != 2 or len(add.outputs) != 1 or not all(conv_ok(c) for c in convs): continue
            by_out = {c.outputs[0].name: c for c in convs}
            x0, x1 = add.inputs
            if x0.name not in by_out or x0 is x1: continue
            if n_conv == 2 and x1.name not in by_out: continue
            ordered = [by_out[x0.name]] + ([by_out[x1.name]] if n_conv == 2 else [])
            if not all(only_feeds(c.outputs[0], add) for c in convs): continue
            relu = relu_after(add, j + 1)
            if relu is None: continue
            unwritten = (_out_cfg(add, 0), _in_cfg(relu, 0))
            between = [_out_cfg(c, 0) for c in convs] + [_in_cfg(add, 0), _in_cfg(add, 1)]
            if not through(*unwritten, *between): return None
            members = list(operations[i:j + 2])
            if not hooks_ok(members, unwritten): return None
            return EpilogueGroup('P2', members, ordered, add, relu)
        return None

    def try_p1(i):
        conv = operations[i]
        if not conv_ok(conv): return None
        relu = relu_after(conv, i + 1)
        if relu is None: return None
        unwritten = (_out_cfg(conv, 0), _in_cfg(relu, 0))
        if not through(*unwritten) or not hooks_ok([conv, relu], unwritten): return None
        return EpilogueGroup('P1', [conv, relu], [conv], None, relu)

    groups, i = [], 0
    while i < len(operations):
        g = try_p2(i) if operations[i].type == 'Conv' else None
        if g is None and operations[i].type == 'Conv': g = try_p1(i)
        if g is None:
            i += 1
            continue
        groups.append(g)
        i += len(g.ops)
    return groups


class TorchExecutor:
    def __init__(self, graph: BaseGraph, device: str = 'cuda'):
        self._graph = graph
        self._device = device
        self._default_quant_fn = PPQuantFunction
        self.cache_parameter_quantization = False
        self._param_cache: Dict[str, tuple] = {}
        self.fuse_parameter_quantization = True
        self._plans: list = []
        self._plan_signature = None
        self._plan_cache: Dict[tuple, list] = {}
        self._fused: Dict[tuple, torch.Tensor] = {}
        self._delegates: Dict[object, Callable] = {}
        self.fuse_epilogues = True
        self._epilogue_cache: Dict[tuple, dict] = {}
        self.channels_last = False
        for v in graph.variables.values():
            if v.is_parameter and v.value is not None: v.value = v.value.to(device)

    def use_channels_last(self) -> 'TorchExecutor':
        self.channels_last = True
        for v in self._graph.variables.values():
            if v.is_parameter and isinstance(v.value, torch.Tensor) and v.value.dim() == 4:
                v.value = v.value.contiguous(memory_format=torch.channels_last)
        return self

    def _place(self, value: torch.Tensor) -> torch.Tensor:
        value = value.to(self._device)
        if self.channels_last and value.dim() == 4: value = value.contiguous(memory_format=torch.channels_last)
        return value

    def register_quantize_delegate(self, config, delegator: Callable) -> None:
        self._delegates[config] = delegator

    def remove_quantize_delegate(self, config) -> None:
        self._delegates.pop(config, None)

    def quantize_function(self, tensor: torch.Tensor, config=None) -> torch.Tensor:
        if self._delegates and config in self._delegates:
            return self._delegates[config](tensor, config)
        return self._default_quant_fn(tensor, config)

    def forward_with_gradient(self, inputs, output_names: List[str] = None, hooks=None):
        return TorchExecutor.forward.__wrapped__(self, inputs, output_names, hooks)

    def partial_graph_forward(self, operations: List[Operation], feed_dict: Dict[str, torch.Tensor],
                              output_names: List[str], with_gradient: bool = False) -> List[torch.Tensor]:
        if not with_gradient:
            with torch.no_grad(): return self._partial_graph_forward(operations, feed_dict, output_names)
        return self._partial_graph_forward(operations, feed_dict, output_names)

    def _partial_graph_forward(self, operations, feed_dict, output_names):
        g = self._graph
        for name, value in feed_dict.items(): g.variables[name].value = self._place(value)
        results = [None] * len(output_names)
        self._fused_parameters(operations)
        plan, fused_done = self._epilogue_plan(operations, None, output_names), set()
        for op in operations:
            if op.name in fused_done: continue
            grp = plan.get(op.name)
            vals = self._run_epilogue(grp, lambda v: v.value, None) if grp is not None else None
            if vals is not None:
                for m in grp.ops:
                    fused_done.add(m.name)
                    for v in m.outputs:
                        v.value = vals[v.name]
                        if v.name in output_names: results[output_names.index(v.name)] = v.value
                continue
            raw_in = [v.value for v in op.inputs]
            if any(x is None for x in raw_in):
                raise ValueError(f'partial_graph_forward: input of {op.name} was not fed')
            if isinstance(op, QuantableOperation):
                qin = [self._quantize_parameter(v, c) if v.is_parameter else self.quantize_function(x, c)
                       for v, x, c in zip(op.inputs, raw_in, op.config.input_quantization_config)]
            else: qin = raw_in
            outs = _forward(op, qin)
            outs = list(outs) if isinstance(outs, (list, tuple)) else [outs]
            if isinstance(op, QuantableOperation):
                outs = [self.quantize_function(y, c) for y, c in zip(outs, op.config.output_quantization_config)]
            for v, y in zip(op.outputs, outs):
                v.value = y
                if v.name in output_names: results[output_names.index(v.name)] = y
        for v in g.variables.values():
            if not v.is_parameter: v.value = None
        return results

    def _fused_parameters(self, operations=None) -> None:
        self._fused = {}
        if not self.fuse_parameter_quantization or self._default_quant_fn is not PPQuantFunction: return
        from .ffi import FloatingQuantizePlan, LinearQuantizePlan
        todo, sig = [], []
        for op in (self._graph.operations.values() if operations is None else operations):
            if not isinstance(op, QuantableOperation): continue
            for v, c in zip(op.inputs, op.config.input_quantization_config):
                if not (v.is_parameter and isinstance(v.value, torch.Tensor) and v.value.is_cuda): continue
                if not QuantizationStates.is_activated(c.state) or c in self._delegates: continue
                pol = c.policy
                floating = pol.has_property(P.FLOATING)
                if not (pol.has_property(P.LINEAR) or floating) or pol.has_property(P.DYNAMIC): continue
                if v.value.dtype != torch.float32 or v.value.requires_grad or v.value.numel() == 0: continue
                if not (isinstance(c.scale, torch.Tensor) and isinstance(c.offset, torch.Tensor)): continue
                axis = c.channel_axis if pol.has_property(P.PER_CHANNEL) else None
                if not LinearQuantizePlan.accepts(v.value, c.scale, c.offset, axis): continue
                rnd = int(getattr(c.rounding, 'value', c.rounding))
                todo.append((v, c, axis, rnd, floating))
                sig.append((v.name, id(c), v.value.data_ptr(), c.scale.data_ptr(), c.offset.data_ptr(), tuple(v.value.shape), c.scale.numel(),
                            axis, c.quant_min, c.quant_max, rnd, floating,
                            (c.exponent_bits, c.mantissa_bits) if floating else None))
        if not todo:
            self._plans, self._plan_signature = [], None
            return
        cached = self._plan_cache.get(tuple(sig))
        if cached is not None:
            self._plan_cache[tuple(sig)] = self._plan_cache.pop(tuple(sig))
            self._plans, self._plan_signature = cached, sig
        if sig != self._plan_signature:
            groups: Dict[tuple, list] = {}
            for item in todo: groups.setdefault((item[3], item[4]), []).append(item)
            self._plans = []
            for (rnd, floating), items in groups.items():
                if floating:
                    plan = FloatingQuantizePlan([(v.value, c.scale, c.offset, axis, c.exponent_bits, c.mantissa_bits,
                                                  c.quant_min, c.quant_max) for v, c, axis, _, _ in items], rounding=rnd)
                else:
                    plan = LinearQuantizePlan([(v.value, c.scale, c.offset, axis, c.quant_min, c.quant_max)
                                               for v, c, axis, _, _ in items], rounding=rnd)
                self._plans.append((plan, [(v.name, id(c)) for v, c, _, _, _ in items]))
            self._plan_signature = sig
            if len(self._plan_cache) >= 8: self._plan_cache.pop(next(iter(self._plan_cache)))
            self._plan_cache[tuple(sig)] = self._plans
        for plan, keys in self._plans:
            for key, out in zip(keys, plan.run()): self._fused[key] = out

    def _epilogue_plan(self, operations: List[Operation], hooks, output_names) -> Dict[str, EpilogueGroup]:
        if not self.fuse_epilogues or torch.is_grad_enabled() or self._default_quant_fn is not PPQuantFunction: return {}
        states = tuple(c.state for op in operations if isinstance(op, QuantableOperation)
                       for c in (*op.config.input_quantization_config, *op.config.output_quantization_config))
        sig = (tuple(op.name for op in operations), tuple((k, id(h)) for k, h in hooks.items()) if hooks else (),
               tuple(output_names or ()), tuple(id(c) for c in self._delegates), states)
        plan = self._epilogue_cache.get(sig)
        if plan is None:
            delegates = self._delegates

            def passes_through(c): return not QuantizationStates.is_activated(c.state) and c not in delegates
            groups = plan_epilogues(operations, hooks, set(self._graph.outputs) | set(output_names or ()), passes_through)
            plan = {g.ops[0].name: g for g in groups}
            if len(self._epilogue_cache) >= 8: self._epilogue_cache.pop(next(iter(self._epilogue_cache)))
            self._epilogue_cache[sig] = plan
        return plan

    def _run_epilogue(self, grp: EpilogueGroup, raw_of: Callable, hooks) -> Optional[Dict[str, torch.Tensor]]:
        from .ffi import bias_act_, bias_add_act
        for conv in grp.convs:
            x, w = raw_of(conv.inputs[0]), conv.inputs[1].value
            if not (isinstance(x, torch.Tensor) and x.is_cuda and x.dtype == torch.float32 and x.dim() == 4
                    and isinstance(w, torch.Tensor) and w.dim() == 4): return None
            fmt = torch.channels_last if self.channels_last else torch.contiguous_format
            if not (x.is_contiguous(memory_format=fmt) and w.is_contiguous(memory_format=fmt)): return None
        if grp.add is not None:
            b_var = grp.add.inputs[1]
            if b_var.source_op not in grp.convs:
                b = raw_of(b_var)
                if not (isinstance(b, torch.Tensor) and b.is_cuda and b.dtype == torch.float32): return None
        hooks = hooks or {}
        ys, biases, qins = {}, {}, {}
        for conv in grp.ops[:len(grp.convs)]:
            raw_in = [raw_of(v) for v in conv.inputs]
            qin, in_cfgs = raw_in, None
            if isinstance(conv, QuantableOperation):
                in_cfgs = list(conv.config.input_quantization_config)
                qin = [self._quantize_parameter(v, c) if v.is_parameter else self.quantize_function(x, c)
                       for v, x, c in zip(conv.inputs, raw_in, in_cfgs)]
            hook = hooks.get(conv.name)
            if hook is not None: qin = hook.pre_forward_hook(inputs=raw_in, quant_inputs=qin, quant_configs=in_cfgs)
            a = conv.attributes
            ys[conv.name] = F.conv2d(qin[0], qin[1], None, stride=a.get('strides', 1), padding=a.get('pads', 0),
                                     groups=a.get('group', 1))
            biases[conv.name] = qin[2]
            qins[conv.name] = qin
        if grp.kind == 'P1':
            conv = grp.convs[0]
            y = ys[conv.name]
            if not bias_act_(y, biases[conv.name], relu=True):
                y.add_(biases[conv.name].view(1, -1, 1, 1)).relu_()
            tail = {conv.name: y, grp.relu.name: y}
        else:
            conv_a = grp.convs[0]
            a = ys[conv_a.name]
            conv_b = grp.convs[1] if len(grp.convs) > 1 else None
            b = ys[conv_b.name] if conv_b is not None else raw_of(grp.add.inputs[1])
            out = bias_add_act(a, biases[conv_a.name], b, biases[conv_b.name] if conv_b is not None else None, relu=True)
            if out is None:
                a.add_(biases[conv_a.name].view(1, -1, 1, 1))
                if conv_b is not None: b.add_(biases[conv_b.name].view(1, -1, 1, 1))
                out = F.relu(a + b)
            tail = {conv_a.name: a, grp.add.name: out, grp.relu.name: out}
            if conv_b is not None: tail[conv_b.name] = b
        values: Dict[str, torch.Tensor] = {}
        for op in grp.ops:
            hook = hooks.get(op.name)
            quantable = isinstance(op, QuantableOperation)
            if op.type != 'Conv':
                raw_in = [values[v.name] if v.name in values else raw_of(v) for v in op.inputs]
                qin, in_cfgs = raw_in, None
                if quantable:
                    in_cfgs = list(op.config.input_quantization_config)
                    qin = [self.quantize_function(x, c) for x, c in zip(raw_in, in_cfgs)]
                if hook is not None: hook.pre_forward_hook(inputs=raw_in, quant_inputs=qin, quant_configs=in_cfgs)
            outs = fp_outs = [tail[op.name]]
            out_cfgs = None
            if quantable:
                out_cfgs = list(op.config.output_quantization_config)
                outs = [self.quantize_function(y, c) for y, c in zip(outs, out_cfgs)]
            if hook is not None:
                outs = hook.post_forward_hook(outputs=fp_outs, quant_outputs=outs, quant_configs=out_cfgs)
            for v, y in zip(op.outputs, outs): values[v.name] = y
        return values

    def _quantize_parameter(self, var: Variable, config) -> torch.Tensor:
        hit = self._fused.get((var.name, id(config)))
        if hit is not None: return hit
        """A parameter and its scale do not change between calibration forwards, so its fake-quantised
        value is computed once and kept resident (the reference recomputes it every forward until
        ParameterBakingPass; same values, ppq/executor/torch.py:516-518).  The cache entry is keyed on
        the identity + version of value, scale and offset and on the config state."""
        if not self.cache_parameter_quantization or not QuantizationStates.is_activated(config.state):
            return self.quantize_function(var.value, config)
        key = (var.value.data_ptr(), var.value._version, id(config.scale), config.scale._version,
               id(config.offset), config.offset._version, int(getattr(config.state, 'value', config.state)))
        hit = self._param_cache.get(var.name)
        if hit is not None and hit[0] == key: return hit[1]
        q = self.quantize_function(var.value, config)
        self._param_cache[var.name] = (key, q)
        return q

    @ torch.no_grad()
    def forward_cached(self, inputs, output_names: List[str], cache: Dict[str, torch.Tensor]) -> List[torch.Tensor]:
        g = self._graph
        if isinstance(inputs, torch.Tensor): inputs = {next(iter(g.inputs)): inputs}
        elif isinstance(inputs, (list, tuple)): inputs = {k: v for k, v in zip(g.inputs, inputs)}
        for name, value in inputs.items():
            if name not in cache: cache[name] = self._place(value)
        need, stack = set(), [g.variables[n] for n in output_names]
        while stack:
            v = stack.pop()
            if v.name in cache or v.is_parameter: continue
            op = v.source_op
            if op is None: raise ValueError(f'forward_cached: graph input {v.name} was not fed')
            if op.name in need: continue
            need.add(op.name)
            stack.extend(op.inputs)
        ops = [op for op in g.topological_sort() if op.name in need]
        if ops: self._fused_parameters(ops)
        plan, fused_done = (self._epilogue_plan(ops, None, output_names) if ops else {}), set()
        for op in ops:
            if op.name in fused_done: continue
            grp = plan.get(op.name)
            vals = (self._run_epilogue(grp, lambda v: v.value if v.is_parameter else cache[v.name], None)
                    if grp is not None else None)
            if vals is not None:
                hidden = grp.relu.inputs[0].name
                for m in grp.ops:
                    fused_done.add(m.name)
                    for v in m.outputs:
                        if v.name != hidden: cache[v.name] = vals[v.name]
                continue
            raw_in = [v.value if v.is_parameter else cache[v.name] for v in op.inputs]
            if isinstance(op, QuantableOperation):
                qin = [self._quantize_parameter(v, c) if v.is_parameter else self.quantize_function(x, c)
                       for v, x, c in zip(op.inputs, raw_in, op.config.input_quantization_config)]
            else: qin = raw_in
            outs = _forward(op, qin)
            outs = list(outs) if isinstance(outs, (list, tuple)) else [outs]
            if isinstance(op, QuantableOperation):
                outs = [self.quantize_function(y, c) for y, c in zip(outs, op.config.output_quantization_config)]
            for v, y in zip(op.outputs, outs): cache[v.name] = y
        return [cache[n] for n in output_names]

    @ torch.no_grad()
    def forward(self, inputs, output_names: List[str] = None, hooks: Dict[str, object] = None) -> List[torch.Tensor]:
        g = self._graph
        if isinstance(inputs, torch.Tensor): inputs = {next(iter(g.inputs)): inputs}
        elif isinstance(inputs, (list, tuple)): inputs = {k: v for k, v in zip(g.inputs, inputs)}
        for name, value in inputs.items(): g.variables[name].value = self._place(value)
        stop_early = output_names is not None and not hooks
        if output_names is None: output_names = list(g.outputs)
        results = [None] * len(output_names)
        visited = set()
        self._fused_parameters()
        ops = g.topological_sort()
        plan, fused_done = self._epilogue_plan(ops, hooks, output_names), set()

        def finish(op, outs):
            for v, y in zip(op.outputs, outs):
                v.value = y
                if v.name in output_names: results[output_names.index(v.name)] = y
            visited.add(op.name)
            for v in op.inputs:
                if not v.is_parameter and all(d.name in visited for d in v.dest_ops): v.value = None

        for op in ops:
            if op.name in fused_done: continue
            grp = plan.get(op.name)
            vals = self._run_epilogue(grp, lambda v: v.value, hooks) if grp is not None else None
            if vals is not None:
                for m in grp.ops:
                    fused_done.add(m.name)
                    finish(m, [vals[v.name] for v in m.outputs])
                if stop_early and all(r is not None for r in results): break
                continue
            hook = hooks.get(op.name) if hooks else None
            raw_in = [v.value for v in op.inputs]
            qin = raw_in
            quantable = isinstance(op, QuantableOperation)
            if quantable:
                in_cfgs = list(op.config.input_quantization_config)
                qin = [self._quantize_parameter(v, c) if v.is_parameter else self.quantize_function(x, c)
                       for v, x, c in zip(op.inputs, raw_in, in_cfgs)]
            if hook is not None:
                qin = hook.pre_forward_hook(inputs=raw_in, quant_inputs=qin, quant_configs=in_cfgs)
            outs = _forward(op, qin)
            outs = list(outs) if isinstance(outs, (list, tuple)) else [outs]
            fp_outs = outs
            if quantable:
                out_cfgs = list(op.config.output_quantization_config)
                outs = [self.quantize_function(y, c) for y, c in zip(outs, out_cfgs)]
            if hook is not None:
                outs = hook.post_forward_hook(outputs=fp_outs, quant_outputs=outs, quant_configs=out_cfgs)
            finish(op, outs)
            if stop_early and all(r is not None for r in results): break
        for v in g.variables.values():
            if not v.is_parameter: v.value = None
        return results


def quantize_graph(graph: BaseGraph, activation_algorithm: str = 'kl', per_channel_weight: bool = True,
                   symmetrical: bool = True, weight_symmetrical: bool = True, num_of_bits: int = 8,
                   hist_bins: int = None, fp8: bool = False, passive_bias: bool = False) -> None:
    qmin, qmax = (-(2 ** (num_of_bits - 1)), 2 ** (num_of_bits - 1) - 1) if symmetrical else (0, 2 ** num_of_bits - 1)
    wmin, wmax = (-(2 ** (num_of_bits - 1)), 2 ** (num_of_bits - 1) - 1) if weight_symmetrical else (0, 2 ** num_of_bits - 1)

    def act_cfg():
        if fp8:
            from .core import FloatingQuantizationConfig
# ... 277 lines not shown
```

### ppq_amd/observer.py

```python
from typing import Dict, List, Optional, Sequence, Tuple

import weakref

import numpy as np
import torch

from .core import (OBSERVER_FLOATING_MSE_FETCHES, OBSERVER_ISOTONE_OBSERVER_AXIS, OBSERVER_KL_HIST_BINS, OBSERVER_KL_HIST_BINS_MANUL_OVERRIDE,
                   OBSERVER_MIN_SCALE, OBSERVER_MIN_SCALE_MANUL_OVERRIDE, OBSERVER_MSE_HIST_BINS,
                   OBSERVER_PERCENTILE, OBSERVER_PERCENTILE_MANUL_OVERRIDE, is_initial, set_activated)
from .core import QuantizationProperty as P
from .core import RoundingPolicy
from .ffi import CUDA, quantile_hint
from .round import ppq_numerical_round, ppq_round_to_power_of_2


def minmax_to_scale_offset(min_val: float, max_val: float, config,
                           scale_threshold: float = OBSERVER_MIN_SCALE) -> Tuple[float, float]:
    if OBSERVER_MIN_SCALE_MANUL_OVERRIDE in config.detail:
        scale_threshold = config.detail[OBSERVER_MIN_SCALE_MANUL_OVERRIDE]
    scale, offset = 1, 0
    if min_val > 0: min_val = 0
    if max_val < 0: max_val = 0
    if config.policy.has_property(P.ASYMMETRICAL):
        range = float(max_val - min_val)
# ... 30 lines not shown
            offset = np.rint(((-lo) / scale.astype(np.float32)).astype(np.float64))
        return scale.tolist(), [int(v) for v in offset.tolist()]
    if config.policy.has_property(P.SYMMETRICAL):
        a, b = np.abs(hi), np.abs(lo)
        m = np.where(b > a, b, a)
        scale = 2 * m.astype(np.float64) / levels
        scale = np.where(scale_threshold > scale, scale_threshold, scale)
        return scale.tolist(), [0] * int(scale.size)
    raise TypeError('Tensor Min Max Observer Excepts either ASYMMETRICAL or SYMMETRICAL quantization config.')


_DEFERRED_SETS: Optional[list] = None


def _set_per_tensor(config, scale: float, offset: float, device) -> None:
    if _DEFERRED_SETS is not None:
        _DEFERRED_SETS.append((config, scale, offset, device))
        return
    config.scale = torch.tensor([scale], dtype=torch.float32, device=device).squeeze(0)
    config.offset = torch.tensor([offset], dtype=torch.float32, device=device).squeeze(0)
    set_activated(config)


def _flush_deferred_sets(pending: list) -> None:
    by_dev: Dict[object, list] = {}
    for item in pending: by_dev.setdefault(torch.device(item[3]), []).append(item)
    for dev, items in by_dev.items():
        chunks = [np.asarray(v, dtype=np.float32).reshape(-1) for _, s, o, _ in items for v in (s, o)]
        flat = torch.from_numpy(np.concatenate(chunks)).to(dev)
        pos = 0
        for k, (config, s, _, _) in enumerate(items):
            if isinstance(s, (list, tuple)):
                C = len(s)
                config.scale, config.offset = flat[pos: pos + C], flat[pos + C: pos + 2 * C]
                pos += 2 * C
            else:
                config.scale, config.offset = flat[pos], flat[pos + 1]
                pos += 2
            set_activated(config)


class ObservationQueue:
    def __init__(self, max_pending_bytes: int = 4 << 30):
        self._minmax = []
        self._minmax_c = []
        self._hist = {}
        self._quantile = {}
        self._bytes = 0
        self._max = max_pending_bytes
        self.launches = 0
        self.recorder: Optional[list] = None

    def __len__(self):
        return (len(self._minmax) + len(self._minmax_c) + sum(len(v) for v in self._hist.values())
                + sum(len(v) for v in self._quantile.values()))

    def _grow(self, value) -> None:
        self._bytes += value.numel() * 4
        if self._bytes > self._max: self.flush()

    def add_minmax(self, value: torch.Tensor, slots: torch.Tensor) -> None:
        self._minmax.append((value, slots))
        self._grow(value)

    def add_minmax_c(self, value: torch.Tensor, channel_axis: int, mins: torch.Tensor, maxs: torch.Tensor, fresh: bool) -> None:
        if any(m.data_ptr() == mins.data_ptr() for _, _, m, _, _ in self._minmax_c): self.flush()
        self._minmax_c.append((value, channel_axis, mins, maxs, bool(fresh)))
        self._grow(value)

    def add_hist(self, value: torch.Tensor, rows: torch.Tensor, asymmetric: bool, p0: float, p1: float = 0.0) -> None:
        self._hist.setdefault((bool(asymmetric), rows.shape[1], value.device), []).append((value, rows, p0, p1))
        self._grow(value)

    def add_quantile(self, value: torch.Tensor, q: float, hint: Optional[torch.Tensor] = None) -> torch.Tensor:
        dest = torch.empty(2, dtype=torch.float32, device=value.device)
        self._quantile.setdefault((float(q), value.device), []).append((value, dest, hint))
        self._grow(value)
        return dest

    def flush(self) -> None:
        if self._quantile:
            pending, self._quantile = self._quantile, {}
            for (q, _), items in pending.items():
                hints, seen = [h for _, _, h in items], set()
                for k in range(len(hints) - 1, -1, -1):
                    if hints[k] is None: continue
                    key = hints[k].data_ptr()
                    if key in seen: hints[k] = None
                    else: seen.add(key)
                CUDA.Quantile_Multi([v for v, _, _ in items], q, [d for _, d, _ in items], hints)
                self.launches += 1
        if self._minmax:
            by_dev = {}
            for v, sl in self._minmax: by_dev.setdefault(v.device, []).append((v, sl))
            self._minmax = []
            for items in by_dev.values():
                CUDA.MinMax_T_Slots_Multi([v for v, _ in items], [sl for _, sl in items])
                self.launches += 1
        if self._minmax_c:
            by_dev = {}
            for it in self._minmax_c: by_dev.setdefault(it[0].device, []).append(it)
            self._minmax_c = []
            for dev, items in by_dev.items():
                CUDA.MinMax_C_Multi([i[0] for i in items], [i[1] for i in items], [i[2] for i in items],
                                    [i[3] for i in items], [i[4] for i in items])
                self.launches += 1
        if self._hist:
            pending, self._hist = self._hist, {}
            for (asym, _, _), items in pending.items():
                vs, rows = [i[0] for i in items], [i[1] for i in items]
                if asym:
                    CUDA.Histogram_Asymmetric_T_Rows_Multi([i[2] for i in items], [i[3] for i in items], vs, rows)
                else:
                    CUDA.Histogram_T_Rows_Multi(vs, rows, [i[2] for i in items])
                self.launches += 1
        self._bytes = 0


SIBLING_PREFETCH = False
_LIVE_OBSERVERS: "weakref.WeakSet" = weakref.WeakSet()
_PREFETCHING = False


def _prefetch_siblings(ob) -> None:
    global _PREFETCHING
    if not SIBLING_PREFETCH or _PREFETCHING: return
    _PREFETCHING = True
    try:
        def device_of(o):
            t = getattr(o, '_hist', None) if getattr(o, '_hist', None) is not None else getattr(o, '_range', None)
            return None if t is None else t.device
        dev = device_of(ob)
        sibs = [o for o in list(_LIVE_OBSERVERS) if isinstance(o, TorchMinMaxObserver) and is_initial(o._quant_cfg) and device_of(o) == dev]
        if ob not in sibs: sibs.append(ob)
        _prefetch(sibs)
    finally:
        _PREFETCHING = False


class BaseTensorObserver:
    queue: Optional[ObservationQueue] = None

    def __init__(self, watch_on, quant_cfg):
        self._watch_on = watch_on
        self._quant_cfg = quant_cfg
        _LIVE_OBSERVERS.add(self)

    def _drain(self) -> None:
        if self.queue is not None and len(self.queue): self.queue.flush()

    def observe(self, value):
        raise NotImplementedError('Implement this function first.')

    def render_quantization_config(self):
        raise NotImplementedError('Implement this function first.')

    def __str__(self) -> str:
        return ('PPQ Tensor Observer (' + self.__class__.__name__ + ') mount on variable ' +
                getattr(self._watch_on, 'name', str(self._watch_on)) + ' observing algorithm: ' +
                str(self._quant_cfg.observer_algorithm))

    def report(self) -> str:
        return ''

    def pending_range(self) -> Optional[torch.Tensor]:
        return None

    def take_range(self, host: np.ndarray) -> None:
        """Receive the host copy of ``pending_range()`` (fetched for all observers at once)."""

    def reducible(self) -> List[Tuple[torch.Tensor, str]]:
        return []

    def gatherable(self) -> List[torch.Tensor]:
        return []

    def take_gathered(self, merged: List[torch.Tensor]) -> None:
        pass


_RANGE_SEEDS: Dict[object, tuple] = {}


def _range_seed(device) -> tuple:
    hit = _RANGE_SEEDS.get(device)
    if hit is None:
        one = torch.tensor([float('inf'), float('-inf')], dtype=torch.float32, device=device)
        hit = _RANGE_SEEDS[device] = (one, one.repeat(CUDA.minmax_slots(), 1).contiguous())
    return hit


class TorchMinMaxObserver(BaseTensorObserver):
    def __init__(self, watch_on, quant_cfg):
        super().__init__(watch_on, quant_cfg)
        self._range: Optional[torch.Tensor] = None
        self._slots: Optional[torch.Tensor] = None
        self._slots_dirty = False
        self._queued_c = False
        self._host_range: Optional[np.ndarray] = None
        self._observed = False

    @ torch.no_grad()
    def observe(self, value: torch.Tensor):
        assert isinstance(value, torch.Tensor), 'TorchMinMaxObserver can only deal with torch Tensor values'
        assert value.numel() > 0, (f'You are observing an empty tensor({getattr(self._watch_on, "name", "")}).')
        if not is_initial(self._quant_cfg): return
        cfg = self._quant_cfg
        if cfg.policy.has_property(P.PER_TENSOR):
            if self._range is None:
                seed = _range_seed(value.device)
                self._range = seed[0].clone()
                self._slots = seed[1].clone()
            if self.queue is not None and value.is_cuda: self.queue.add_minmax(value, self._slots)
            else: CUDA.MinMax_T_Slots(value, self._slots)
            self._slots_dirty = True
        elif cfg.policy.has_property(P.PER_CHANNEL):
            queued = (self.queue is not None and value.is_cuda and CUDA.minmax_c_outer_is_one(value, cfg.channel_axis))
            fresh = False
            if self._range is None:
                C = value.shape[cfg.channel_axis]
                self._range = torch.empty((2, C), dtype=torch.float32, device=value.device)
                fresh = queued and CUDA.minmax_c_fresh_ok(value, cfg.channel_axis)
                if not fresh: self._range[0].fill_(float('inf')); self._range[1].fill_(float('-inf'))
            if queued:
                self.queue.add_minmax_c(value, cfg.channel_axis, self._range[0], self._range[1], fresh)
                self._queued_c = True
            else: CUDA.MinMax_C(value, cfg.channel_axis, self._range[0], self._range[1])
        else:
            raise TypeError('Min-max Observer only work with per-tensor or per-channel quantize policy.')
        self._observed = True
        self._host_range = None

    def _fold(self) -> None:
        if self._queued_c:
            self._drain()
            self._queued_c = False
        if self._slots_dirty:
            self._drain()
            CUDA.MinMax_Slots_Finish(self._slots, self._range)
            self._slots_dirty = False

    def pending_range(self):
        if not (is_initial(self._quant_cfg) and self._observed): return None
        self._fold()
        return self._range

    def take_range(self, host: np.ndarray) -> None:
        self._host_range = host

    def reducible(self):
        if self._range is None: return []
        self._fold()
        if self._range.ndim == 1: return [(self._range[0:1], 'min'), (self._range[1:2], 'max')]
        return [(self._range[0], 'min'), (self._range[1], 'max')]

    def _range_on_host(self) -> np.ndarray:
        if not self._observed:
            raise ValueError('Can not render quantization config yet, Observer data collator is empty. '
                             'Invoke observe() function before render config.')
        if self._host_range is None: _prefetch_siblings(self)
        if self._host_range is None:
            self._fold()
            self._host_range = self._range.cpu().numpy()
        return self._host_range

    def render_quantization_config(self):
        if not is_initial(self._quant_cfg): return
        cfg = self._quant_cfg
        r = self._range_on_host()
        device = self._range.device
        if cfg.policy.has_property(P.PER_TENSOR):
            scale, offset = minmax_to_scale_offset(min_val=float(r[0]), max_val=float(r[1]), config=cfg)
            _set_per_tensor(cfg, scale, offset, device)
        elif cfg.policy.has_property(P.PER_CHANNEL):
            scales, offsets = minmax_to_scale_offset_channels(np.ascontiguousarray(r[0]), np.ascontiguousarray(r[1]), cfg)
            if _DEFERRED_SETS is not None:
                _DEFERRED_SETS.append((cfg, scales, offsets, device))
                return
            cfg.scale = torch.tensor(scales, dtype=torch.float32, device=device)
            cfg.offset = torch.tensor(offsets, dtype=torch.float32, device=device)
            set_activated(cfg)
        else:
            raise TypeError('Min-max Observer only work with per-tensor or per-channel quantize policy.')


class TorchHistObserver(TorchMinMaxObserver):
    def __init__(self, watch_on, quant_cfg, hist_bins: int = OBSERVER_KL_HIST_BINS):
        self._phase = 'Detecting Minmax'
        self._hist = None
        self._rows = None
        self._rows_dirty = False
        self._hist_scale = None
        self._min = None
        self._max = None
        self._losses: Optional[np.ndarray] = None
        if OBSERVER_KL_HIST_BINS_MANUL_OVERRIDE in quant_cfg.detail:
            hist_bins = quant_cfg.detail[OBSERVER_KL_HIST_BINS_MANUL_OVERRIDE]
        self._hist_bins = hist_bins
        super().__init__(watch_on, quant_cfg)

    def observe(self, value: torch.Tensor):
        if not is_initial(self._quant_cfg): return
        assert value.numel() > 0, (f'You are observing an empty tensor({getattr(self._watch_on, "name", "")}).')
        if self._phase == 'Detecting Minmax':
            if self.queue is not None and self.queue.recorder is not None and value.is_cuda:
                self.queue.recorder.append((self, value))
            return super().observe(value)
        elif self._phase == 'Collating Hist':
            self._losses = None
            if getattr(self, '_best', None) is not None: self._best = None
            if self._hist is None:
                self._hist = torch.zeros(size=(self._hist_bins,), dtype=torch.int32, device=value.device)
                if self._hist_bins <= 16384:
                    self._rows = torch.zeros(size=(CUDA.hist_rows(), self._hist_bins), dtype=torch.int32,
                                             device=value.device)
            if self._quant_cfg.policy.has_property(P.ASYMMETRICAL):
                if self._rows is not None:
                    if self.queue is not None: self.queue.add_hist(value, self._rows, True, self._min, self._max)
                    else: CUDA.Histogram_Asymmetric_T_Rows(self._min, self._max, tensor=value, rows=self._rows)
                    self._rows_dirty = True
                else:
                    CUDA.Histogram_Asymmetric_T(self._min, self._max, tensor=value, histogram=self._hist)
            elif self._quant_cfg.policy.has_property(P.SYMMETRICAL):
                if self._rows is not None:
                    if self.queue is not None: self.queue.add_hist(value, self._rows, False, self._hist_scale)
                    else: CUDA.Histogram_T_Rows(tensor=value, rows=self._rows, scale=self._hist_scale)
                    self._rows_dirty = True
                else:
                    CUDA.Histogram_T(tensor=value, histogram=self._hist, scale=self._hist_scale)
            else:
                raise TypeError('Quantization Property is invalid, expect either ASYMMETRICAL or SYMMETRICAL config here.')

    def pending_range(self):
        return super().pending_range() if self._phase == 'Detecting Minmax' else None

    def _fold_hist(self) -> None:
        if self._rows_dirty:
            self._drain()
            CUDA.Histogram_Rows_Finish(self._rows, self._hist)
            self._rows_dirty = False
            if self._rows.is_cuda: self._rows.record_stream(torch.cuda.current_stream(self._rows.device))
            self._rows = None

    def histogram(self) -> Optional[torch.Tensor]:
        self._fold_hist()
        return self._hist

    def reducible(self):
        if self._phase == 'Detecting Minmax': return super().reducible()
        return [(self.histogram(), 'sum')] if self._hist is not None else []

    search_kind = 'kl'

    def search_key(self):
        return ('kl', self._hist_bins, self._quant_cfg.num_of_bits)

    def take_losses(self, losses: np.ndarray) -> None:
        self._losses = losses

    def hist_to_scale_offset(self, histogram: torch.Tensor, hist_bins: int, hist_scale: float, config,
                             scale_threshold: float = OBSERVER_MIN_SCALE) -> Tuple[float, int]:
        if config.policy.has_property(P.ASYMMETRICAL):
            raise PermissionError('KL observer is not designed for ASYMMETRICAL quantization')
        if OBSERVER_MIN_SCALE_MANUL_OVERRIDE in config.detail:
            scale_threshold = config.detail[OBSERVER_MIN_SCALE_MANUL_OVERRIDE]
        quant_bins = 2 ** (config.num_of_bits - 1)
        if self._losses is None: _prefetch_siblings(self)
        if self._losses is None:
            self._losses = CUDA.KLLosses(histogram, config.num_of_bits).cpu().numpy()[0]
        losses = [{'kl': float(kl), 'bin_range': (j + 1) * quant_bins} for j, kl in enumerate(self._losses)]
        best_bin_range = sorted(losses, key=lambda x: x['kl'])[0]['bin_range']
        scale, offset = (best_bin_range / self._hist_bins) * hist_scale * (self._hist_bins / quant_bins), 0
        scale = max(scale, scale_threshold)
        if config.policy.has_property(P.POWER_OF_2):
            scale = ppq_round_to_power_of_2(scale, policy=RoundingPolicy.ROUND_HALF_UP)
        return scale, offset

    def render_quantization_config(self):
        if not is_initial(self._quant_cfg): return
        if not self._quant_cfg.policy.has_property(P.PER_TENSOR):
            raise ValueError('Hist observer can only apply with per-tensor quantization config.')
        if self._phase == 'Detecting Minmax':
            r = self._range_on_host()
            min_val, max_val = float(r[0]), float(r[1])
            if self._quant_cfg.policy.has_property(P.SYMMETRICAL):
                hist_range = float(max(abs(max_val), abs(min_val)))
            else:
                hist_range = max_val - min_val
            self._min = min_val
            self._max = max_val
            self._hist_scale = hist_range / self._hist_bins
            self._phase = 'Collating Hist'
        elif self._phase == 'Collating Hist':
            if self._hist is None:
                raise ValueError('Can not render quantization config yet, histogram is empty. '
                                 'Invoke observe() function before render config.')
            scale, offset = self.hist_to_scale_offset(histogram=self.histogram(), hist_bins=self._hist_bins,
                                                      hist_scale=self._hist_scale, config=self._quant_cfg)
            _set_per_tensor(self._quant_cfg, scale, offset, self._hist.device)


class ChannelwiseKLObserver(TorchHistObserver):
    def __init__(self, watch_on, quant_cfg, hist_bins: int = OBSERVER_KL_HIST_BINS):
        super().__init__(watch_on, quant_cfg, hist_bins)
        if not quant_cfg.policy.has_property(P.PER_CHANNEL) or not quant_cfg.policy.has_property(P.SYMMETRICAL):
            raise TypeError('ChannelwiseKLObserver needs a symmetrical per-channel config.')
        self._scales_dev: Optional[torch.Tensor] = None

    def observe(self, value: torch.Tensor):
        if not is_initial(self._quant_cfg): return
        assert value.numel() > 0, (f'You are observing an empty tensor({getattr(self._watch_on, "name", "")}).')
        if self._phase == 'Detecting Minmax':
            return TorchMinMaxObserver.observe(self, value)
        C = value.shape[self._quant_cfg.channel_axis]
        if self._hist is None:
            self._hist = torch.zeros(size=(C, self._hist_bins), dtype=torch.int32, device=value.device)
        CUDA.Histogram_C_Scales(value, self._quant_cfg.channel_axis, self._hist, self._scales_dev)

    def histogram(self): return self._hist

    def render_quantization_config(self):
        cfg = self._quant_cfg
        if not is_initial(cfg): return
        if self._phase == 'Detecting Minmax':
            r = self._range_on_host()
            hs = [float(max(abs(float(hi)), abs(float(lo)))) / self._hist_bins for lo, hi in zip(r[0], r[1])]
            self._hist_scale = hs
            self._scales_dev = torch.tensor(hs, dtype=torch.float32, device=self._range.device)
            self._phase = 'Collating Hist'
            return
        if self._hist is None:
            raise ValueError('Can not render quantization config yet, histogram is empty. '
                             'Invoke observe() function before render config.')
        losses = CUDA.KLLosses(self._hist, cfg.num_of_bits).cpu().numpy()
        scales = []
        for c in range(self._hist.shape[0]):
            self._losses = losses[c]
            scale, _ = self.hist_to_scale_offset(self._hist[c], self._hist_bins, self._hist_scale[c], cfg)
            scales.append(scale)
        self._losses = None
        cfg.scale = torch.tensor(scales, dtype=torch.float32, device=self._hist.device)
        cfg.offset = torch.zeros(len(scales), dtype=torch.float32, device=self._hist.device)
        set_activated(cfg)


class TorchPercentileObserver(BaseTensorObserver):
    def __init__(self, watch_on, quant_cfg):
        super().__init__(watch_on, quant_cfg)
        if OBSERVER_PERCENTILE_MANUL_OVERRIDE not in quant_cfg.detail:
            self._percentile = OBSERVER_PERCENTILE
        else: self._percentile = quant_cfg.detail[OBSERVER_PERCENTILE_MANUL_OVERRIDE]
        self._percentile_collector = []
        self._sum: Optional[torch.Tensor] = None
        self._hint: Optional[torch.Tensor] = None

    @ torch.no_grad()
    def observe(self, value: torch.Tensor):
        if not is_initial(self._quant_cfg): return
        assert value is not None, ('You are observing an Empty Tensor. '
                                   '(This Error is usually due to you have a wrong Quantizer configuration.)')
        assert value.numel() > 0, (f'You are observing an empty tensor({getattr(self._watch_on, "name", "")}).')
        assert isinstance(value, torch.Tensor), 'TorchMinMaxObserver can only deal with torch Tensor values'
        if self._quant_cfg.policy.has_property(P.PER_TENSOR):
            if value.is_cuda and (self._hint is None or self._hint.device != value.device):
                self._hint = quantile_hint(value.device)
            if self.queue is not None and value.is_cuda:
                self._percentile_collector.append(self.queue.add_quantile(value, self._percentile, self._hint).view(1, -1))
            else:
                self._percentile_collector.append(CUDA.Quantile_Hinted(value, self._percentile, self._hint).view(1, -1))
        elif self._quant_cfg.policy.has_property(P.PER_CHANNEL):
            raise PermissionError('Percentile observer can not deal with per channel quantization.')
        else:
            raise TypeError('Min-max Observer only work with per-tensor or per-channel quantize policy.')

    def _fold(self):
        self._drain()
        if self._percentile_collector:
            stacked = torch.cat(self._percentile_collector, dim=0).float()
            part = torch.cat([stacked.sum(dim=0), stacked.new_tensor([float(stacked.shape[0])])])
            self._sum = part if self._sum is None else self._sum + part
            self._percentile_collector = []

    def reducible(self):
        self._fold()
# ... 504 lines not shown
```

Measured before the change: 3549 samples/s.

## Fuse min/max and histogram observation into bias+ReLU epilogue kernels

Adds epilogue kernels that, besides applying bias, residual add and ReLU, also accumulate per-tensor min/max slots or histogram rows for the observed outputs in the same pass. The executor picks observers whose per-tensor targets can be fused, passes their slots or rows to the kernel, and marks the tensor as claimed so the later observe call skips its separate queued reduction. This avoids re-reading large activation tensors for calibration statistics, at the cost of more register and LDS pressure in the epilogue and a more complex claim protocol between executor and observers.

```diff
diff --git a/include/ppq_hip.h b/include/ppq_hip.h
--- a/include/ppq_hip.h
+++ b/include/ppq_hip.h
@@ -225,6 +225,22 @@
                     int relu, void* stream);
 int ppqhip_bias_add_act(float* a, const float* bias_a, float* b, const float* bias_b, float* out,
                         int64_t n, int64_t num_channel, int64_t elem_per_channel, int relu, void* stream);
+
+#define PPQHIP_NOT_FUSED 1
+#define PPQHIP_EP_STATS_FORCE 1
+#define PPQHIP_EP_STATS_SMALL_GRID 2
+typedef struct ppqhip_ep_stat {
+    float* slots;
+    int32_t* rows;
+    float p0, p1;
+} ppqhip_ep_stat;
+int ppqhip_bias_act_stats(float* y, const float* bias, int64_t n, int64_t num_channel, int64_t elem_per_channel,
+                          int relu, const ppqhip_ep_stat* stat_y, int asymmetric, int clip_outliers,
+                          int64_t num_bins, int flags, void* stream);
+int ppqhip_bias_add_act_stats(float* a, const float* bias_a, float* b, const float* bias_b, float* out,
+                              int64_t n, int64_t num_channel, int64_t elem_per_channel, int relu,
+                              const ppqhip_ep_stat* stats, int asymmetric, int clip_outliers, int64_t num_bins,
+                              int flags, void* stream);
 
 typedef struct ppqhip_adaround_job {
     const float* w;
diff --git a/ppq_amd/_lib.py b/ppq_amd/_lib.py
--- a/ppq_amd/_lib.py
+++ b/ppq_amd/_lib.py
@@ -38,6 +38,9 @@
     'ppqhip_lsq_finish_multi': (c_int, [c_vp, c_int, c_vp]),
     'ppqhip_bias_act': (c_int, [c_f32p, c_f32p, c_i64, c_i64, c_i64, c_int, c_vp]),
     'ppqhip_bias_add_act': (c_int, [c_f32p, c_f32p, c_f32p, c_f32p, c_f32p, c_i64, c_i64, c_i64, c_int, c_vp]),
+    'ppqhip_bias_act_stats': (c_int, [c_f32p, c_f32p, c_i64, c_i64, c_i64, c_int, c_vp, c_int, c_int, c_i64, c_int, c_vp]),
+    'ppqhip_bias_add_act_stats': (c_int, [c_f32p, c_f32p, c_f32p, c_f32p, c_f32p, c_i64, c_i64, c_i64, c_int, c_vp, c_int,
+                                          c_int, c_i64, c_int, c_vp]),
     'ppqhip_fq_float_t': (c_int, [c_f32p, c_f32p, c_f32p, c_f32p, c_i64, c_int, c_int, c_flt, c_flt, c_int, c_vp]),
     'ppqhip_fq_float_c': (c_int, [c_f32p, c_f32p, c_f32p, c_f32p, c_i64, c_i64, c_i64, c_int, c_int, c_flt, c_flt,
                                   c_int, c_vp]),
diff --git a/ppq_amd/calibration.py b/ppq_amd/calibration.py
--- a/ppq_amd/calibration.py
+++ b/ppq_amd/calibration.py
@@ -29,7 +29,7 @@
                  process_group=None, check_steps: bool = True, async_observe: bool = False,
                  use_hip_graph: bool = False, batch_observations: bool = True,
                  reuse_activations: bool = False, reuse_budget_bytes: int = 64 << 30,
-                 queue_bytes: int = None) -> None:
+                 queue_bytes: int = None, fuse_observations: bool = True) -> None:
         super().__init__(name='PPQ Runtime Calibration Pass')
         self._method = method
         self._observers: Dict[str, OperationObserver] = {}
@@ -44,6 +44,7 @@
         self._queue = None
         self._reuse_activations = reuse_activations
         self._queue_bytes = queue_bytes
+        self._fuse_observations = fuse_observations
         self._reuse_budget = reuse_budget_bytes
         self._replay: list = []
         self._replay_bytes = 0
@@ -160,6 +161,15 @@
 
     def optimize(self, graph, dataloader: Iterable, executor, calib_steps: int = 32,
                  collate_fn: Callable = None, **kwargs) -> None:
+        switch = getattr(executor, 'fuse_observations', None)
+        if switch is not None: executor.fuse_observations = bool(switch and self._fuse_observations)
+        try:
+            self._optimize(graph, dataloader, executor, calib_steps, collate_fn, **kwargs)
+        finally:
+            if switch is not None: executor.fuse_observations = switch
+
+    def _optimize(self, graph, dataloader: Iterable, executor, calib_steps: int = 32,
+                  collate_fn: Callable = None, **kwargs) -> None:
         if collate_fn is not None: self._collate_fn = collate_fn
         if calib_steps is not None: self._calib_steps = calib_steps
         if self._check_steps:
diff --git a/ppq_amd/csrc/common.hpp b/ppq_amd/csrc/common.hpp
--- a/ppq_amd/csrc/common.hpp
+++ b/ppq_amd/csrc/common.hpp
@@ -26,7 +26,7 @@
     K_MINMAX_C, K_MSE_SEARCH, K_KL_LOSSES, K_TENSOR_CLIP, K_ROUNDING_LOSS, K_CHANNEL_SUM, K_FLOAT_SCALE_SEARCH, K_LSQ_FINISH,
     K_ADAROUND_FWD, K_ADAROUND_BWD, K_FETCH_ROWS, K_MEASURE_ROWS, K_MEASURE_FINISH, K_ROUNDTUNE_FWD, K_EQUALIZE_SCALE,
     K_EQUALIZE_APPLY, K_SSD_SCALES, K_SSD_APPLY, K_FQ_MEASURE_ROWS, K_STAT_MOMENTS, K_STAT_SHAPE,
-    K_SPLIT_PLAN, K_SPLIT_APPLY, K_NUM
+    K_SPLIT_PLAN, K_SPLIT_APPLY, K_BIAS_ACT_STATS, K_BIAS_ADD_ACT_STATS, K_NUM
 };
 extern const char* const kKernelNames[K_NUM];
 
diff --git a/ppq_amd/csrc/epilogue.hip b/ppq_amd/csrc/epilogue.hip
--- a/ppq_amd/csrc/epilogue.hip
+++ b/ppq_amd/csrc/epilogue.hip
@@ -1,4 +1,8 @@
+#include <algorithm>
+#include <type_traits>
+
 #include "common.hpp"
+#include "hist_bin.hpp"
 
 namespace ppqhip {
 namespace {
@@ -135,6 +139,236 @@
     return PPQHIP_OK;
 }
 
+constexpr int kEsU = 2;
+constexpr int kEsHistBlock = 512;
+constexpr int kEsHistWgPerCu = 2;
+constexpr int kEsMmBlock = 256;
+constexpr int kEsMmWgPerCu = 8;
+constexpr int kEsMaxBins = 4096;
+constexpr int kEsHistMinTiles = 4;
+constexpr long long kEpStatsMinElems = 1ll << 20;
+
+struct EsTarget {
+    float* slots;
+    int* rows;
+    float a0, hs;
+};
+struct EsArgs {
+    EpArgs ep;
+    EsTarget t[3];
+    int bins;
+    uint32_t tiles;
+};
+
+template <int BLOCK, bool HIST, bool RESID, bool BIAS_B, bool PLANE, bool ASYM, bool CLIP>
+__global__ __launch_bounds__(BLOCK) void epilogue_stats_kernel(const EsArgs q) {
+    extern __shared__ int lds[];
+    constexpr uint32_t TILE = BLOCK * kEsU;
+    constexpr int NB = PLANE ? 1 : 4;
+    const EpArgs& p = q.ep;
+    const uint32_t G = gridDim.x, g = blockIdx.x;
+    uint32_t t, t_end;
+    even_split(q.tiles, G, g, t, t_end);
+    if (t >= t_end) return;
+    float4* a4 = reinterpret_cast<float4*>(p.a);
+    float4* b4 = reinterpret_cast<float4*>(p.b);
+    float4* o4 = reinterpret_cast<float4*>(p.out);
+    const uint32_t full = p.nvec / TILE;
+    const int bins = q.bins;
+    const bool on0 = HIST ? q.t[0].rows != nullptr : q.t[0].slots != nullptr;
+    const bool on1 = RESID && BIAS_B && (HIST ? q.t[1].rows != nullptr : q.t[1].slots != nullptr);
+    const bool on2 = RESID && (HIST ? q.t[2].rows != nullptr : q.t[2].slots != nullptr);
+
+    Binner<ASYM, CLIP, true> acc0, acc1, acc2;
+    float mn0 = INFINITY, mx0 = -INFINITY, mn1 = INFINITY, mx1 = -INFINITY, mn2 = INFINITY, mx2 = -INFINITY;
+    if (HIST) {
+        acc0.init(lds, bins); acc0.set_rule(q.t[0].a0, q.t[0].hs);
+        acc1.init(lds + bins, bins); acc1.set_rule(q.t[1].a0, q.t[1].hs);
+        acc2.init(lds + 2 * bins, bins); acc2.set_rule(q.t[2].a0, q.t[2].hs);
+    }
+
+    struct Tile { float4 a[kEsU], b[kEsU]; float ba[kEsU][NB], bb[kEsU][NB]; };
+    auto bias_of = [&](const float* __restrict__ bias, uint32_t v, float (&out)[NB]) {
+        if (PLANE) out[0] = bias[channel_of(v, p.epc, p.nc)];
+        else {
+#pragma unroll
+            for (int e = 0; e < NB; e++) out[e] = bias[channel_of(v * 4u + e, p.epc, p.nc)];
+        }
+    };
+    auto fetch = [&](Tile& T, uint32_t tile) {
+#pragma unroll
+        for (int k = 0; k < kEsU; k++) {
+            const uint32_t vv = min(tile * TILE + k * BLOCK + threadIdx.x, p.nvec - 1);
+            T.a[k] = a4[vv];
+            bias_of(p.bias_a, vv, T.ba[k]);
+            if (RESID) T.b[k] = b4[vv];
+            if (BIAS_B) bias_of(p.bias_b, vv, T.bb[k]);
+        }
+    };
+    auto bias4_of = [](const float (&v)[NB]) { return PLANE ? make_float4(v[0], v[0], v[0], v[0]) : make_float4(v[0], v[NB > 1 ? 1 : 0], v[NB > 2 ? 2 : 0], v[NB > 3 ? 3 : 0]); };
+    auto stat = [&](auto full_tag, Binner<ASYM, CLIP, true>& acc, float& mn, float& mx, const float4& v, bool in, bool first) {
+        constexpr bool FULL = decltype(full_tag)::value;
+        if (HIST) {
+            int b[4];
+            acc.bins4(v, b);
+            if (first) acc.elect(b[0], in);
+            if (FULL && CLIP) acc.commit4_exec(b);
+            else {
+                acc.template commit<FULL>(b[0], in); acc.template commit<FULL>(b[1], in);
+                acc.template commit<FULL>(b[2], in); acc.template commit<FULL>(b[3], in);
+            }
+        } else if (FULL || in) {
+            mn = fminf(fminf(mn, v.x), fminf(v.y, fminf(v.z, v.w)));
+            mx = fmaxf(fmaxf(mx, v.x), fmaxf(v.y, fmaxf(v.z, v.w)));
+        }
+    };
+    auto consume_as = [&](auto full_tag, const Tile& T, uint32_t tile) {
+        constexpr bool FULL = decltype(full_tag)::value;
+#pragma unroll
+        for (int k = 0; k < kEsU; k++) {
+            const uint32_t vv = tile * TILE + k * BLOCK + threadIdx.x;
+            const bool in = FULL || vv < p.nvec;
+            const float4 x = add4(T.a[k], bias4_of(T.ba[k]));
+            if (!RESID) {
+                const float4 r = act4<true>(x);
+                if (in) a4[vv] = r;
+                if (on0) stat(full_tag, acc0, mn0, mx0, r, in, k == 0);
+                continue;
+            }
+            if (in) a4[vv] = x;
+            float4 y = T.b[k];
+            if (BIAS_B) { y = add4(y, bias4_of(T.bb[k])); if (in) b4[vv] = y; }
+            const float4 o = act4<true>(add4(x, y));
+            if (in) o4[vv] = o;
+            if (on0) stat(full_tag, acc0, mn0, mx0, x, in, k == 0);
+            if (on1) stat(full_tag, acc1, mn1, mx1, y, in, k == 0);
+            if (on2) stat(full_tag, acc2, mn2, mx2, o, in, k == 0);
+        }
+    };
+    auto consume = [&](const Tile& T, uint32_t tile) {
+        if (tile < full) consume_as(std::true_type{}, T, tile);
+        else consume_as(std::false_type{}, T, tile);
+    };
+
+    Tile A, B;
+    fetch(A, t);
+    if (HIST) {
+        for (int i = threadIdx.x; i < (RESID ? 3 : 1) * bins; i += BLOCK) lds[i] = 0;
+        asm volatile("s_waitcnt lgkmcnt(0)\n\ts_barrier" ::: "memory");
+    }
+    for (;;) {
+        fetch(B, min(t + 1, t_end - 1));
+        consume(A, t);
+        if (++t >= t_end) break;
+        fetch(A, min(t + 1, t_end - 1));
+        consume(B, t);
+        if (++t >= t_end) break;
+    }
+
+    if (HIST) {
+        if (on0) acc0.flush_hot();
+        if (on1) acc1.flush_hot();
+        if (on2) acc2.flush_hot();
+        asm volatile("s_waitcnt lgkmcnt(0)" ::: "memory");
+        __syncthreads();
+        for (int b = threadIdx.x; b < bins; b += BLOCK) {
+            if (on0) { const int s = lds[b]; if (s) q.t[0].rows[(size_t)g * bins + b] += s; }
+            if (on1) { const int s = lds[bins + b]; if (s) q.t[1].rows[(size_t)g * bins + b] += s; }
+            if (on2) { const int s = lds[2 * bins + b]; if (s) q.t[2].rows[(size_t)g * bins + b] += s; }
+        }
+    } else {
+        float* red = reinterpret_cast<float*>(lds);
+        constexpr int NW = BLOCK / kWave;
+        mn0 = wave_min(mn0); mx0 = wave_max(mx0);
+        mn1 = wave_min(mn1); mx1 = wave_max(mx1);
+        mn2 = wave_min(mn2); mx2 = wave_max(mx2);
+        const int wid = threadIdx.x >> 6, lane = threadIdx.x & 63;
+        if (lane == 0) {
+            red[0 * NW + wid] = mn0; red[1 * NW + wid] = mx0; red[2 * NW + wid] = mn1;
+            red[3 * NW + wid] = mx1; red[4 * NW + wid] = mn2; red[5 * NW + wid] = mx2;
+        }
+        __syncthreads();
+        if (threadIdx.x == 0) {
+            for (int w = 1; w < NW; w++) {
+                mn0 = fminf(mn0, red[0 * NW + w]); mx0 = fmaxf(mx0, red[1 * NW + w]);
+                mn1 = fminf(mn1, red[2 * NW + w]); mx1 = fmaxf(mx1, red[3 * NW + w]);
+                mn2 = fminf(mn2, red[4 * NW + w]); mx2 = fmaxf(mx2, red[5 * NW + w]);
+            }
+            if (on0) { float* sl = q.t[0].slots + 2 * g; sl[0] = fminf(mn0, sl[0]); sl[1] = fmaxf(mx0, sl[1]); }
+            if (on1) { float* sl = q.t[1].slots + 2 * g; sl[0] = fminf(mn1, sl[0]); sl[1] = fmaxf(mx1, sl[1]); }
+            if (on2) { float* sl = q.t[2].slots + 2 * g; sl[0] = fminf(mn2, sl[0]); sl[1] = fmaxf(mx2, sl[1]); }
+        }
+    }
+}
+
+template <int BLOCK, bool HIST, bool RESID, bool BIAS_B, bool PLANE>
+void launch_stats_rule(const EsArgs& q, int grid, size_t lds, bool asym, bool clip, hipStream_t st) {
+#define PPQ_LAUNCH_ES(A, CL)                                                                                             \
+    hipLaunchKernelGGL((epilogue_stats_kernel<BLOCK, HIST, RESID, BIAS_B, PLANE, A, CL>), dim3(grid), dim3(BLOCK), lds, st, q)
+    if constexpr (!HIST) { PPQ_LAUNCH_ES(false, false); return; }
+    else switch ((asym ? 2 : 0) | (clip ? 1 : 0)) {
+        case 0: PPQ_LAUNCH_ES(false, false); break;
+        case 1: PPQ_LAUNCH_ES(false, true); break;
+        case 2: PPQ_LAUNCH_ES(true, false); break;
+        default: PPQ_LAUNCH_ES(true, true); break;
+    }
+#undef PPQ_LAUNCH_ES
+}
+
+template <bool RESID, bool BIAS_B>
+int launch_stats(EsArgs q, int64_t n, int64_t C, int64_t epc, bool aligned, const ppqhip_ep_stat* stats, int nstats, int relu,
+                 int asym, int clip, int64_t bins, int flags, hipStream_t st, const char* what) {
+    bool hist = false, mm = false;
+    for (int k = 0; k < nstats; k++) {
+        if (!RESID && k > 0) break;
+        if (k == 1 && !BIAS_B) continue;
+        hist = hist || stats[k].rows != nullptr;
+        mm = mm || stats[k].slots != nullptr;
+    }
+    if (hist && mm) { set_error("%s: min/max slots and histogram rows in one launch", what); return PPQHIP_ERR_INVALID_VALUE; }
+    if (!hist && !mm) return PPQHIP_NOT_FUSED;
+    if (!relu || !aligned || (n & 3) != 0 || n > 0x7fffffffLL) return PPQHIP_NOT_FUSED;
+    if (hist && (bins <= 0 || bins > kEsMaxBins)) return PPQHIP_NOT_FUSED;
+    if (!(flags & PPQHIP_EP_STATS_FORCE) && n < kEpStatsMinElems) return PPQHIP_NOT_FUSED;
+    if (int s = validate(n, C, epc, what)) return s;
+    EpArgs& p = q.ep;
+    p.nc = make_fastdiv((uint32_t)C);
+    p.nvec = (uint32_t)(n >> 2);
+    p.tail = p.nvec * 4u;
+    p.ntail = 0;
+    const bool plane = (epc % 4 == 0);
+    p.epc = make_fastdiv((uint32_t)(plane ? epc / 4 : epc));
+    q.bins = hist ? (int)bins : 0;
+    for (int k = 0; k < 3; k++) {
+        EsTarget& d = q.t[k];
+        d.slots = nullptr; d.rows = nullptr; d.a0 = 0.f; d.hs = 1.f;
+        if (k >= nstats || (!RESID && k > 0) || (k == 1 && !BIAS_B)) continue;
+        d.slots = stats[k].slots; d.rows = (int*)stats[k].rows;
+        if (asym) { d.a0 = stats[k].p0; d.hs = (stats[k].p1 - stats[k].p0) / (float)bins; }
+        else d.hs = stats[k].p0;
+    }
+    const uint32_t block = hist ? kEsHistBlock : kEsMmBlock, tile = block * kEsU;
+    q.tiles = (p.nvec + tile - 1) / tile;
+    int64_t grid = hist ? (int64_t)q.tiles / kEsHistMinTiles : (int64_t)q.tiles;
+    const int64_t cap = hist ? std::min<int64_t>((int64_t)num_cu() * kEsHistWgPerCu, ppqhip_hist_rows())
+                             : std::min<int64_t>((int64_t)num_cu() * kEsMmWgPerCu, ppqhip_minmax_slots());
+    if (grid > cap) grid = cap;
+    if ((flags & PPQHIP_EP_STATS_SMALL_GRID) && grid > 2) grid = 2;
+    if (grid < 1) grid = 1;
+    const double bytes = 4.0 * (double)n * (RESID ? (BIAS_B ? 5.0 : 4.0) : 2.0);
+    LaunchScope scope(RESID ? K_BIAS_ADD_ACT_STATS : K_BIAS_ACT_STATS, bytes, st);
+    if (hist) {
+        const size_t lds = sizeof(int) * (RESID ? 3 : 1) * (size_t)bins;
+        if (plane) launch_stats_rule<kEsHistBlock, true, RESID, BIAS_B, true>(q, (int)grid, lds, asym != 0, clip != 0, st);
+        else launch_stats_rule<kEsHistBlock, true, RESID, BIAS_B, false>(q, (int)grid, lds, asym != 0, clip != 0, st);
+    } else {
+        const size_t lds = sizeof(float) * 6 * (kEsMmBlock / kWave);
+        if (plane) launch_stats_rule<kEsMmBlock, false, RESID, BIAS_B, true>(q, (int)grid, lds, false, false, st);
+        else launch_stats_rule<kEsMmBlock, false, RESID, BIAS_B, false>(q, (int)grid, lds, false, false, st);
+    }
+    return finish_launch(what);
+}
+
 }
 }
 
@@ -173,4 +407,27 @@
     return finish_launch("bias_add_act");
 }
 
-}
+int ppqhip_bias_act_stats(float* y, const float* bias, int64_t n, int64_t num_channel, int64_t elem_per_channel, int relu,
+                          const ppqhip_ep_stat* stat_y, int asymmetric, int clip_outliers, int64_t num_bins, int flags,
+                          void* stream) {
+    if (!y || !bias || !stat_y) { set_error("bias_act_stats: null pointer"); return PPQHIP_ERR_INVALID_VALUE; }
+    EsArgs q{};
+    q.ep.a = y; q.ep.bias_a = bias;
+    return launch_stats<false, false>(q, n, num_channel, elem_per_channel, aligned16(y), stat_y, 1, relu, asymmetric, clip_outliers,
+                                      num_bins, flags, (hipStream_t)stream, "bias_act_stats");
+}
+
+int ppqhip_bias_add_act_stats(float* a, const float* bias_a, float* b, const float* bias_b, float* out, int64_t n,
+                              int64_t num_channel, int64_t elem_per_channel, int relu, const ppqhip_ep_stat* stats,
+                              int asymmetric, int clip_outliers, int64_t num_bins, int flags, void* stream) {
+    if (!a || !bias_a || !b || !out || !stats) { set_error("bias_add_act_stats: null pointer"); return PPQHIP_ERR_INVALID_VALUE; }
+    EsArgs q{};
+    q.ep.a = a; q.ep.bias_a = bias_a; q.ep.b = b; q.ep.bias_b = bias_b; q.ep.out = out;
+    const bool aligned = aligned16(a) && aligned16(b) && aligned16(out);
+    if (bias_b) return launch_stats<true, true>(q, n, num_channel, elem_per_channel, aligned, stats, 3, relu, asymmetric,
+                                                clip_outliers, num_bins, flags, (hipStream_t)stream, "bias_add_act_stats");
+    return launch_stats<true, false>(q, n, num_channel, elem_per_channel, aligned, stats, 3, relu, asymmetric, clip_outliers,
+                                     num_bins, flags, (hipStream_t)stream, "bias_add_act_stats");
+}
+
+}
diff --git a/ppq_amd/csrc/hist.hip b/ppq_amd/csrc/hist.hip
--- a/ppq_amd/csrc/hist.hip
+++ b/ppq_amd/csrc/hist.hip
@@ -1,4 +1,5 @@
 #include "common.hpp"
+#include "hist_bin.hpp"
 
 namespace ppqhip {
 
@@ -15,7 +16,6 @@
 constexpr uint32_t kTileElems = kTileVec * 4;
 static_assert(kHistBlock % 64 == 0 && kHistBlock >= 64 && kHistBlock <= 1024, "histogram workgroup: whole waves");
 
-typedef float v2f __attribute__((ext_vector_type(2)));
 
 struct BinRule {
     float a;
@@ -29,63 +29,6 @@
     BinRule r; r.a = a; r.hs = hs; r.rcp = 1.0f / hs; r.bins = bins; r.clip = clip; r.asym = asym;
     return r;
 }
-
-__device__ __forceinline__ bool quotient_is_safe(float t) {
-    return __builtin_fabsf(t - __builtin_rintf(t)) >= __builtin_fabsf(t) * 0x1p-22f;
-}
-
-__device__ __forceinline__ int f2i_abs(float t) {
-    int r;
-    asm("v_cvt_i32_f32_e64 %0, |%1|" : "=v"(r) : "v"(t));
-    return r;
-}
-__device__ __forceinline__ int f2i_floor(float t) {
-    int r;
-    asm("v_cvt_flr_i32_f32 %0, %1" : "=v"(r) : "v"(t));
-    return r;
-}
-
-template <bool ASYM, bool CLIP, bool HOT>
-struct Binner : WaveBinCounter<ASYM, CLIP, HOT> {
-    using Base = WaveBinCounter<ASYM, CLIP, HOT>;
-    using Base::h; using Base::last; using Base::hot_bin; using Base::hot_cnt;
-    float a0, hs, rcp;
-
-    __device__ __forceinline__ void set_rule(float a, float scale) { a0 = a; hs = scale; rcp = 1.0f / scale; }
-
-    __device__ __forceinline__ void bins4(const float4& v, int (&b)[4]) const {
-        v2f x01 = {v.x, v.y}, x23 = {v.z, v.w};
-        if (ASYM) { x01 = x01 - a0; x23 = x23 - a0; }
-        const v2f t01 = x01 * rcp, t23 = x23 * rcp;
-        const v2f r01 = {__builtin_rintf(t01.x), __builtin_rintf(t01.y)};
-        const v2f r23 = {__builtin_rintf(t23.x), __builtin_rintf(t23.y)};
-        const v2f d01 = t01 - r01, d23 = t23 - r23;
-        const v2f e01 = t01 * 0x1p-22f, e23 = t23 * 0x1p-22f;
-        const bool u0 = !(__builtin_fabsf(d01.x) >= __builtin_fabsf(e01.x));
-        const bool u1 = !(__builtin_fabsf(d01.y) >= __builtin_fabsf(e01.y));
-        const bool u2 = !(__builtin_fabsf(d23.x) >= __builtin_fabsf(e23.x));
-        const bool u3 = !(__builtin_fabsf(d23.y) >= __builtin_fabsf(e23.y));
-        b[0] = ASYM ? f2i_floor(t01.x) : f2i_abs(t01.x);
-        b[1] = ASYM ? f2i_floor(t01.y) : f2i_abs(t01.y);
-        b[2] = ASYM ? f2i_floor(t23.x) : f2i_abs(t23.x);
-        b[3] = ASYM ? f2i_floor(t23.y) : f2i_abs(t23.y);
-        if (u0 | u1 | u2 | u3) {
-            if (u0) b[0] = exact_bin(ASYM ? x01.x : __builtin_fabsf(v.x));
-            if (u1) b[1] = exact_bin(ASYM ? x01.y : __builtin_fabsf(v.y));
-            if (u2) b[2] = exact_bin(ASYM ? x23.x : __builtin_fabsf(v.z));
-            if (u3) b[3] = exact_bin(ASYM ? x23.y : __builtin_fabsf(v.w));
-        }
-    }
-    __device__ __forceinline__ int exact_bin(float a) const { return f2i_sat(__builtin_floorf(a / hs)); }
-
-    __device__ __forceinline__ int bin1(float v) const {
-        const float a = ASYM ? (v - a0) : __builtin_fabsf(v);
-        const float t = a * rcp;
-        if (quotient_is_safe(t)) return ASYM ? f2i_floor(t) : f2i_abs(t);
-        return exact_bin(a);
-    }
-
-};
 
 constexpr int kReduceBins = 32, kReduceSlices = 32, kReduceBlock = kReduceBins * kReduceSlices;
 __global__ __launch_bounds__(kReduceBlock) void hist_reduce_kernel(const int* __restrict__ partial, int count, int bins,
diff --git a/ppq_amd/csrc/hist_bin.hpp b/ppq_amd/csrc/hist_bin.hpp
--- /dev/null
+++ b/ppq_amd/csrc/hist_bin.hpp
@@ -0,0 +1,66 @@
+#pragma once
+
+#include "common.hpp"
+
+namespace ppqhip {
+
+typedef float v2f __attribute__((ext_vector_type(2)));
+
+__device__ __forceinline__ bool quotient_is_safe(float t) {
+    return __builtin_fabsf(t - __builtin_rintf(t)) >= __builtin_fabsf(t) * 0x1p-22f;
+}
+
+__device__ __forceinline__ int f2i_abs(float t) {
+    int r;
+    asm("v_cvt_i32_f32_e64 %0, |%1|" : "=v"(r) : "v"(t));
+    return r;
+}
+__device__ __forceinline__ int f2i_floor(float t) {
+    int r;
+    asm("v_cvt_flr_i32_f32 %0, %1" : "=v"(r) : "v"(t));
+    return r;
+}
+
+template <bool ASYM, bool CLIP, bool HOT>
+struct Binner : WaveBinCounter<ASYM, CLIP, HOT> {
+    using Base = WaveBinCounter<ASYM, CLIP, HOT>;
+    using Base::h; using Base::last; using Base::hot_bin; using Base::hot_cnt;
+    float a0, hs, rcp;
+
+    __device__ __forceinline__ void set_rule(float a, float scale) { a0 = a; hs = scale; rcp = 1.0f / scale; }
+
+    __device__ __forceinline__ void bins4(const float4& v, int (&b)[4]) const {
+        v2f x01 = {v.x, v.y}, x23 = {v.z, v.w};
+        if (ASYM) { x01 = x01 - a0; x23 = x23 - a0; }
+        const v2f t01 = x01 * rcp, t23 = x23 * rcp;
+        const v2f r01 = {__builtin_rintf(t01.x), __builtin_rintf(t01.y)};
+        const v2f r23 = {__builtin_rintf(t23.x), __builtin_rintf(t23.y)};
+        const v2f d01 = t01 - r01, d23 = t23 - r23;
+        const v2f e01 = t01 * 0x1p-22f, e23 = t23 * 0x1p-22f;
+        const bool u0 = !(__builtin_fabsf(d01.x) >= __builtin_fabsf(e01.x));
+        const bool u1 = !(__builtin_fabsf(d01.y) >= __builtin_fabsf(e01.y));
+        const bool u2 = !(__builtin_fabsf(d23.x) >= __builtin_fabsf(e23.x));
+        const bool u3 = !(__builtin_fabsf(d23.y) >= __builtin_fabsf(e23.y));
+        b[0] = ASYM ? f2i_floor(t01.x) : f2i_abs(t01.x);
+        b[1] = ASYM ? f2i_floor(t01.y) : f2i_abs(t01.y);
+        b[2] = ASYM ? f2i_floor(t23.x) : f2i_abs(t23.x);
+        b[3] = ASYM ? f2i_floor(t23.y) : f2i_abs(t23.y);
+        if (u0 | u1 | u2 | u3) {
+            if (u0) b[0] = exact_bin(ASYM ? x01.x : __builtin_fabsf(v.x));
+            if (u1) b[1] = exact_bin(ASYM ? x01.y : __builtin_fabsf(v.y));
+            if (u2) b[2] = exact_bin(ASYM ? x23.x : __builtin_fabsf(v.z));
+            if (u3) b[3] = exact_bin(ASYM ? x23.y : __builtin_fabsf(v.w));
+        }
+    }
+    __device__ __forceinline__ int exact_bin(float a) const { return f2i_sat(__builtin_floorf(a / hs)); }
+
+    __device__ __forceinline__ int bin1(float v) const {
+        const float a = ASYM ? (v - a0) : __builtin_fabsf(v);
+        const float t = a * rcp;
+        if (quotient_is_safe(t)) return ASYM ? f2i_floor(t) : f2i_abs(t);
+        return exact_bin(a);
+    }
+
+};
+
+}
diff --git a/ppq_amd/csrc/runtime.hip b/ppq_amd/csrc/runtime.hip
--- a/ppq_amd/csrc/runtime.hip
+++ b/ppq_amd/csrc/runtime.hip
@@ -32,7 +32,7 @@
     "minmax_c", "mse_search", "kl_losses", "tensor_clip", "rounding_loss", "channel_sum", "float_scale_search", "lsq_finish",
     "adaround_fwd", "adaround_bwd", "fetch_rows", "measure_rows", "measure_finish", "roundtune_fwd", "equalize_scale",
     "equalize_apply", "ssd_scales", "ssd_apply", "fq_measure_rows", "stat_moments", "stat_shape",
-    "split_plan", "split_apply"};
+    "split_plan", "split_apply", "bias_act_stats", "bias_add_act_stats"};
 
 int num_cu() {
     static std::mutex mu;
diff --git a/ppq_amd/ffi.py b/ppq_amd/ffi.py
--- a/ppq_amd/ffi.py
+++ b/ppq_amd/ffi.py
@@ -1,3 +1,4 @@
+import ctypes
 import threading
 import weakref
 from typing import List
@@ -183,6 +184,71 @@
         _raise(lib.ppqhip_bias_add_act(a.data_ptr(), bias_a.data_ptr(), b.data_ptr(), 0 if bias_b is None else bias_b.data_ptr(),
                                        out.data_ptr(), a.numel(), geo[0], geo[1], 1 if relu else 0, _stream()))
     return out
+
+
+
+EP_STATS_FORCE = 1
+EP_STATS_SMALL_GRID = 2
+EP_NOT_FUSED = 1
+
+
+class _EpStat(ctypes.Structure):
+    _fields_ = [('slots', ctypes.c_void_p), ('rows', ctypes.c_void_p), ('p0', ctypes.c_float), ('p1', ctypes.c_float)]
+
+
+def _ep_stats(targets, device):
+    recs = (_EpStat * len(targets))()
+    mode = None
+    for rec, t in zip(recs, targets):
+        if t is None: continue
+        if t[0] == 'minmax':
+            slots = t[1]
+            _f32(slots, 'Slots')
+            if slots.numel() != 2 * lib.ppqhip_minmax_slots() or not slots.is_contiguous() or slots.device != device:
+                raise RuntimeError(_KERNEL_FAILURE + f'slots must be a contiguous [{lib.ppqhip_minmax_slots()}, 2] tensor on {device}')
+            key = ('minmax', False, True, 0)
+            rec.slots = slots.data_ptr()
+        elif t[0] == 'hist':
+            _, rows, asym, p0, p1, clip = t
+            _check(rows, torch.int32, 'Rows(Expect to be INT32)')
+            if rows.ndim != 2 or rows.shape[0] != lib.ppqhip_hist_rows() or not rows.is_contiguous() or rows.device != device:
+                raise RuntimeError(_KERNEL_FAILURE + f'rows must be a contiguous [{lib.ppqhip_hist_rows()}, bins] tensor on {device}')
+            key = ('hist', bool(asym), bool(clip), int(rows.shape[1]))
+            rec.rows, rec.p0, rec.p1 = rows.data_ptr(), float(p0), float(p1)
+        else:
+            raise ValueError(f'unknown statistics target {t[0]!r}')
+        if mode is not None and key != mode:
+            raise ValueError(f'statistics targets of one launch must be of one kind: {mode} and {key}')
+        mode = key
+    if mode is None: mode = ('minmax', False, True, 0)
+    return recs, int(mode[1]), int(mode[2]), mode[3]
+
+
+def _fused(status: int) -> bool:
+    if status == EP_NOT_FUSED: return False
+    _raise(status)
+    return True
+
+
+def bias_act_stats_(y: torch.Tensor, bias: torch.Tensor, target, flags: int = 0) -> bool:
+    geo = _epilogue_geometry([y], [bias])
+    if geo is None or target is None: return False
+    recs, asym, clip, bins = _ep_stats([target], y.device)
+    with _DeviceOf(y):
+        return _fused(lib.ppqhip_bias_act_stats(y.data_ptr(), bias.data_ptr(), y.numel(), geo[0], geo[1], 1, ctypes.addressof(recs),
+                                                asym, clip, bins, int(flags), _stream()))
+
+
+def bias_add_act_stats(a: torch.Tensor, bias_a: torch.Tensor, b: torch.Tensor, bias_b, targets, flags: int = 0):
+    geo = _epilogue_geometry([a, b], [bias_a] if bias_b is None else [bias_a, bias_b])
+    if geo is None or a.data_ptr() == b.data_ptr() or len(targets) != 3 or all(t is None for t in targets): return None
+    recs, asym, clip, bins = _ep_stats(list(targets), a.device)
+    out = torch.empty_like(a)
+    with _DeviceOf(a):
+        ok = _fused(lib.ppqhip_bias_add_act_stats(a.data_ptr(), bias_a.data_ptr(), b.data_ptr(), 0 if bias_b is None else bias_b.data_ptr(),
+                                                  out.data_ptr(), a.numel(), geo[0], geo[1], 1, ctypes.addressof(recs), asym, clip, bins,
+                                                  int(flags), _stream()))
+    return out if ok else None
 
 
 _ADAROUND_JOB = np.dtype([('w', '<u8'), ('v', '<u8'), ('scale', '<u8'), ('offset', '<u8'), ('out', '<u8'), ('dy', '<u8'),
diff --git a/ppq_amd/harness.py b/ppq_amd/harness.py
--- a/ppq_amd/harness.py
+++ b/ppq_amd/harness.py
@@ -144,10 +144,11 @@
 
 
 class EpilogueGroup:
-    __slots__ = ('kind', 'ops', 'convs', 'add', 'relu')
+    __slots__ = ('kind', 'ops', 'convs', 'add', 'relu', 'observed')
 
     def __init__(self, kind, ops, convs, add, relu):
         self.kind, self.ops, self.convs, self.add, self.relu = kind, ops, convs, add, relu
+        self.observed = None
 
     def __repr__(self): return f'{self.kind}({", ".join(op.name for op in self.ops)})'
 
@@ -236,6 +237,39 @@
     return groups
 
 
+def plan_fused_observations(group: EpilogueGroup, hooks: Dict[str, object] = None) -> Dict[str, object]:
+    from .observer import CalibrationHook, TorchHistObserver, TorchMinMaxObserver, TorchMSEObserver
+    from .core import is_initial
+    hooks = hooks or {}
+    relu_out = group.relu.outputs[0].name
+    written = {relu_out: None}
+    if group.kind == 'P2':
+        for conv in group.convs: written[conv.outputs[0].name] = None
+    member_hooks = [(op, hooks.get(op.name)) for op in group.ops]
+    if any(h is not None and (type(h) is not CalibrationHook or h.stream is not None) for _, h in member_hooks):
+        return written
+    tensor_of = {v: v for v in written}
+    hidden = group.relu.inputs[0].name
+    tensor_of[hidden] = relu_out
+    watchers: Dict[str, list] = {v: [] for v in written}
+    for op, h in member_hooks:
+        if h is None or not isinstance(op, QuantableOperation): continue
+        shown = list(zip(op.outputs, op.config.output_quantization_config))
+        if op.type != 'Conv': shown += list(zip(op.inputs, op.config.input_quantization_config))
+        for var, cfg in shown:
+            key = tensor_of.get(var.name)
+            ob = h._observer_table.get(cfg)
+            if key is not None and ob is not None and not any(ob is w for w in watchers[key]): watchers[key].append(ob)
+    for key, obs in watchers.items():
+        if len(obs) != 1: continue
+        ob = obs[0]
+        if type(ob) not in (TorchMinMaxObserver, TorchHistObserver, TorchMSEObserver): continue
+        cfg = ob._quant_cfg
+        if not is_initial(cfg) or not cfg.policy.has_property(P.PER_TENSOR): continue
+        written[key] = ob
+    return written
+
+
 class TorchExecutor:
     def __init__(self, graph: BaseGraph, device: str = 'cuda'):
         self._graph = graph
@@ -251,6 +285,8 @@
         self._delegates: Dict[object, Callable] = {}
         self.fuse_epilogues = True
         self._epilogue_cache: Dict[tuple, dict] = {}
+        self.fuse_observations = True
+        self.fuse_observations_min_elems = None
         self.channels_last = False
         for v in graph.variables.values():
             if v.is_parameter and v.value is not None: v.value = v.value.to(device)
@@ -386,8 +422,21 @@
             self._epilogue_cache[sig] = plan
         return plan
 
+    def _fused_targets(self, grp: EpilogueGroup, hooks, device) -> Dict[str, tuple]:
+        if not self.fuse_observations or not hooks: return {}
+        if grp.observed is None: grp.observed = plan_fused_observations(grp, hooks)
+        out, kind = {}, None
+        for name, ob in grp.observed.items():
+            if ob is None or ob.queue is None: continue
+            target = ob.fused_target(device)
+            if target is None: continue
+            key = (target[0], target[1].shape[1], target[2], target[5]) if target[0] == 'hist' else ('minmax',)
+            if kind is None: kind = key
+            if key == kind: out[name] = (ob, target)
+        return out
+
     def _run_epilogue(self, grp: EpilogueGroup, raw_of: Callable, hooks) -> Optional[Dict[str, torch.Tensor]]:
-        from .ffi import bias_act_, bias_add_act
+        from .ffi import EP_STATS_FORCE, bias_act_, bias_act_stats_, bias_add_act, bias_add_act_stats
         for conv in grp.convs:
             x, w = raw_of(conv.inputs[0]), conv.inputs[1].value
             if not (isinstance(x, torch.Tensor) and x.is_cuda and x.dtype == torch.float32 and x.dim() == 4
@@ -415,10 +464,19 @@
                                      groups=a.get('group', 1))
             biases[conv.name] = qin[2]
             qins[conv.name] = qin
+        first = ys[grp.convs[0].name]
+        fused = self._fused_targets(grp, hooks, first.device)
+        flags = 0
+        if fused and self.fuse_observations_min_elems is not None:
+            if first.numel() < self.fuse_observations_min_elems: fused = {}
+            flags = EP_STATS_FORCE
+        relu_out = grp.relu.outputs[0].name
         if grp.kind == 'P1':
             conv = grp.convs[0]
             y = ys[conv.name]
-            if not bias_act_(y, biases[conv.name], relu=True):
+            if relu_out in fused and bias_act_stats_(y, biases[conv.name], fused[relu_out][1], flags):
+                fused[relu_out][0].claim(y)
+            elif not bias_act_(y, biases[conv.name], relu=True):
                 y.add_(biases[conv.name].view(1, -1, 1, 1)).relu_()
             tail = {conv.name: y, grp.relu.name: y}
         else:
@@ -426,7 +484,16 @@
             a = ys[conv_a.name]
             conv_b = grp.convs[1] if len(grp.convs) > 1 else None
             b = ys[conv_b.name] if conv_b is not None else raw_of(grp.add.inputs[1])
-            out = bias_add_act(a, biases[conv_a.name], b, biases[conv_b.name] if conv_b is not None else None, relu=True)
+            out = None
+            if fused:
+                names = (conv_a.outputs[0].name, conv_b.outputs[0].name if conv_b is not None else None, relu_out)
+                out = bias_add_act_stats(a, biases[conv_a.name], b, biases[conv_b.name] if conv_b is not None else None,
+                                         [fused[n][1] if n in fused else None for n in names], flags)
+                if out is not None:
+                    for n, t in zip(names, (a, b, out)):
+                        if n in fused: fused[n][0].claim(t)
+            if out is None:
+                out = bias_add_act(a, biases[conv_a.name], b, biases[conv_b.name] if conv_b is not None else None, relu=True)
             if out is None:
                 a.add_(biases[conv_a.name].view(1, -1, 1, 1))
                 if conv_b is not None: b.add_(biases[conv_b.name].view(1, -1, 1, 1))
diff --git a/ppq_amd/observer.py b/ppq_amd/observer.py
--- a/ppq_amd/observer.py
+++ b/ppq_amd/observer.py
@@ -206,6 +206,20 @@
     def observe(self, value):
         raise NotImplementedError('Implement this function first.')
 
+    _claimed = None
+
+    def fused_target(self, device):
+        return None
+
+    def claim(self, value) -> None:
+        self._claimed = value
+
+    def _take_claim(self, value) -> bool:
+        c = self._claimed
+        if c is None: return False
+        self._claimed = None
+        return c is value or (c.data_ptr() == value.data_ptr() and c.shape == value.shape and c.stride() == value.stride())
+
     def render_quantization_config(self):
         raise NotImplementedError('Implement this function first.')
 
@@ -265,7 +279,8 @@
                 seed = _range_seed(value.device)
                 self._range = seed[0].clone()
                 self._slots = seed[1].clone()
-            if self.queue is not None and value.is_cuda: self.queue.add_minmax(value, self._slots)
+            if self._take_claim(value): pass
+            elif self.queue is not None and value.is_cuda: self.queue.add_minmax(value, self._slots)
             else: CUDA.MinMax_T_Slots(value, self._slots)
             self._slots_dirty = True
         elif cfg.policy.has_property(P.PER_CHANNEL):
@@ -285,6 +300,15 @@
         self._observed = True
         self._host_range = None
 
+    def fused_target(self, device):
+        if not is_initial(self._quant_cfg) or not self._quant_cfg.policy.has_property(P.PER_TENSOR): return None
+        if self._range is None:
+            seed = _range_seed(device)
+            self._range = seed[0].clone()
+            self._slots = seed[1].clone()
+        if self._slots is None or self._slots.device != device: return None
+        return ('minmax', self._slots)
+
     def _fold(self) -> None:
         if self._queued_c:
             self._drain()
@@ -363,11 +387,10 @@
         elif self._phase == 'Collating Hist':
             self._losses = None
             if getattr(self, '_best', None) is not None: self._best = None
-            if self._hist is None:
-                self._hist = torch.zeros(size=(self._hist_bins,), dtype=torch.int32, device=value.device)
-                if self._hist_bins <= 16384:
-                    self._rows = torch.zeros(size=(CUDA.hist_rows(), self._hist_bins), dtype=torch.int32,
-                                             device=value.device)
+            self._alloc_hist(value.device)
+            if self._rows is not None and self._take_claim(value):
+                self._rows_dirty = True
+                return
             if self._quant_cfg.policy.has_property(P.ASYMMETRICAL):
                 if self._rows is not None:
                     if self.queue is not None: self.queue.add_hist(value, self._rows, True, self._min, self._max)
@@ -384,6 +407,22 @@
                     CUDA.Histogram_T(tensor=value, histogram=self._hist, scale=self._hist_scale)
             else:
                 raise TypeError('Quantization Property is invalid, expect either ASYMMETRICAL or SYMMETRICAL config here.')
+
+    def _alloc_hist(self, device) -> None:
+        if self._hist is None:
+            self._hist = torch.zeros(size=(self._hist_bins,), dtype=torch.int32, device=device)
+            if self._hist_bins <= 16384:
+                self._rows = torch.zeros(size=(CUDA.hist_rows(), self._hist_bins), dtype=torch.int32, device=device)
+
+    def fused_target(self, device):
+        if self._phase == 'Detecting Minmax': return super().fused_target(device)
+        cfg = self._quant_cfg
+        if self._phase != 'Collating Hist' or not is_initial(cfg) or not cfg.policy.has_property(P.PER_TENSOR): return None
+        self._alloc_hist(device)
+        if self._rows is None or self._rows.device != device: return None
+        if cfg.policy.has_property(P.ASYMMETRICAL): return ('hist', self._rows, True, self._min, self._max, True)
+        if cfg.policy.has_property(P.SYMMETRICAL): return ('hist', self._rows, False, self._hist_scale, 0.0, True)
+        return None
 
     def pending_range(self):
         return super().pending_range() if self._phase == 'Detecting Minmax' else None
```

New measurement: 3408 samples/s. 0.96x the previous value.
